# AntonXue/nn-sdp

Hardware: NVIDIA B200
Metric: queries/sec (clique LMI blocks assembled: value * cliques_per_query) (higher is better)
Workload: dtype f64

## Files before the change

### nn-sdp_b200/csrc/api.cu

```cuda
#include <math.h>
#include <stdarg.h>
#include <stdio.h>
#include <stdlib.h>
#include <string.h>

#include <algorithm>
#include <cmath>
#include <condition_variable>
#include <deque>
#include <functional>
#include <memory>
#include <mutex>
#include <thread>
#include <unordered_map>

#include <cuda.h>

#include "internal.h"

namespace nnsdp {

static thread_local std::string g_err;

void set_error(const char* fmt, ...) {
// ... 22 lines not shown
namespace {

struct DevBuf {
  void* p = nullptr;
  size_t cap = 0;
  int32_t ensure(size_t bytes) {
    if (bytes <= cap && p) return NNSDP_OK;
    if (p) cudaFree(p);
    p = nullptr;
    cap = 0;
    if (bytes == 0) bytes = 8;
    NN_CUDA(cudaMalloc(&p, bytes));
    cap = bytes;
    return NNSDP_OK;
  }
  void release() {
    if (p) cudaFree(p);
    p = nullptr;
    cap = 0;
  }
  template <class T>
  T* as() const {
    return reinterpret_cast<T*>(p);
  }
};

struct NetPerDev {
  int dev = -1;
  std::vector<DevBuf> M, Wt;
  DevBuf n, off, xoff, blk_of, Mptr, Wtptr, ldT, bias;
  NetDev nd{};
  void release() {
    for (auto& x : M) x.release();
    for (auto& x : Wt) x.release();
    n.release(); off.release(); xoff.release(); blk_of.release();
    Mptr.release(); Wtptr.release(); ldT.release(); bias.release();
  }
};

int round_up(int64_t v, int64_t m) { return (int)(((v + m - 1) / m) * m); }

}

struct nnsdp_net {
  nnsdp_ctx* ctx = nullptr;
  Shape sh;
  std::vector<int> ldT;
  std::vector<NetPerDev> per;
  int64_t max_block = 0;
  struct Cached {
    int dev_index;
    int64_t beta, Qcap, ring;
    int dense;
    nnsdp_batch* b;
  };
  mutable std::mutex cache_mu;
  mutable std::vector<Cached> cache;
};

namespace {

enum Stage {
  ST_BOUNDS = 0, ST_PREP = 1, ST_GRAM = 2, ST_EMIT = 3, ST_D2H = 4,
  ST_EMIT_FILL = 5, ST_EMIT_WINDOW = 6, ST_EMIT_EDGE = 7,
  ST_COUNT = 8
};

struct StageSpan {
  int stage;
  cudaEvent_t e0, e1;
};

}

namespace {

class WorkerPool {
 public:
  explicit WorkerPool(int n) {
    for (int i = 0; i < n; ++i) th_.emplace_back([this] { loop(); });
  }
  ~WorkerPool() {
    {
      std::lock_guard<std::mutex> l(m_);
      stop_ = true;
    }
    cv_.notify_all();
    for (auto& t : th_) t.join();
  }
  void submit(int group, std::function<void()> fn) {
    {
      std::lock_guard<std::mutex> l(m_);
      if ((int)pending_.size() <= group) pending_.resize(group + 1, 0);
      ++pending_[group];
      q_.emplace_back(group, std::move(fn));
    }
    cv_.notify_one();
  }
  void wait_group(int group) {
    std::unique_lock<std::mutex> l(m_);
    done_cv_.wait(l, [&] { return (int)pending_.size() <= group || pending_[group] == 0; });
  }
  void wait_all() {
    std::unique_lock<std::mutex> l(m_);
    done_cv_.wait(l, [&] {
      for (int p : pending_)
        if (p) return false;
      return true;
    });
    pending_.clear();
  }
  int size() const { return (int)th_.size(); }

 private:
  void loop() {
    for (;;) {
      std::pair<int, std::function<void()>> job;
      {
        std::unique_lock<std::mutex> l(m_);
        cv_.wait(l, [&] { return stop_ || !q_.empty(); });
        if (stop_ && q_.empty()) return;
        job = std::move(q_.front());
        q_.pop_front();
      }
      job.second();
      {
        std::lock_guard<std::mutex> l(m_);
        --pending_[job.first];
      }
      done_cv_.notify_all();
    }
  }
  std::vector<std::thread> th_;
  std::deque<std::pair<int, std::function<void()>>> q_;
  std::vector<int> pending_;
  std::mutex m_;
  std::condition_variable cv_, done_cv_;
  bool stop_ = false;
};

constexpr int GATHER_STAGES = 4;

}

struct nnsdp_batch {
  GatherPlan gp;
  std::vector<CliqueRanges> mats_host;
  DevBuf d_thin_idx, d_packed;
  double* h_packed = nullptr;
  size_t h_packed_doubles = 0;
  cudaEvent_t ev_packed[GATHER_STAGES] = {nullptr, nullptr, nullptr, nullptr};
  std::unique_ptr<WorkerPool> pool;
  std::vector<int> h_cnt;
  std::vector<int> h_pairs;
  std::vector<int64_t> pair_begin;
  DevBuf d_pairs;
  int64_t gather_bytes_dma = 0, gather_bytes_zeroed = 0, gather_bytes_thin = 0;
  nnsdp_ctx* ctx = nullptr;
  int dev_index = 0, dev = 0;
  const nnsdp_net* net = nullptr;
  const NetPerDev* nd = nullptr;
  int64_t beta = 0, Qcap = 0, ring = 0, Q = 0;
  bool dense = false;
  bool packed = false;
  PackedLayout lay;
  DevBuf d_bands;
  DevBuf d_tmaps, d_tmap_ok;
  int nbands = 0, band_max_m = 0;
  int64_t emitted_bytes = 0, packed_present_cells = 0;
  int64_t ring_zeroed = 0;
  std::vector<uint8_t> slot_bulk;
  std::vector<int> bulk_begin;
  std::vector<int64_t> bulk_entries;
  int64_t pass_entries = 0;
  std::vector<BulkItem> sel;
  std::vector<CholFront> chol;
  DevBuf d_chol;
  DevBuf ze_netv, ze_g, ze_rows, ze_part, ze_io, ze_err;
  nnsdp_sizes sz{};
  PlanHost plan;
  DevBuf d_tiles, d_strips, d_bulk, d_mats, d_panel, d_goff, d_ldG;
  std::vector<long long> goff;
  std::vector<int> ldG;
  long long gram_per_query = 0;
  DevBuf x1min, x1max, ymin, ymax, smin, smax, gin, gbnd, gsec, outS, outvec, outinvP, gout;
  DevBuf xmin, xmax, acxmin, acxmax, smin_c, smax_c;
  DevBuf d11, Md, T0, Bt, u, aff, part, act, cnt, Z11, Z1K, U;
  DevBuf gram, ringbuf, flags;
  DevBuf cr_rowsA, cr_rowsB, cr_bias, cr_prel, cr_preu, cr_du, cr_bu, cr_dl;
  DevBuf cr_keep_l, cr_keep_u;
  bool keep_preact = false, preact_valid = false;
  BatchDev bd{};
  GramDev gd{};
  PlanDev pd{};
  bool have_inputs = false, bounds_supplied = false, bounds_done = false, prepared = false;
  bool shared_gram = false;
  int bounds_method = 0;
  cudaStream_t st = nullptr, st_copy = nullptr;
  cudaEvent_t ev_start = nullptr, ev_stop = nullptr;
  cudaEvent_t ev_done[2] = {nullptr, nullptr}, ev_free[2] = {nullptr, nullptr};
  std::vector<StageSpan> spans;
  std::vector<cudaEvent_t> ev_pool;
  float stage_ms[ST_COUNT] = {};
  int64_t stage_launches[ST_COUNT] = {};

  cudaEvent_t get_event() {
    if (!ev_pool.empty()) {
      cudaEvent_t e = ev_pool.back();
      ev_pool.pop_back();
      return e;
    }
    cudaEvent_t e = nullptr;
    cudaEventCreate(&e);
    return e;
  }
  bool span_open = false;
  void span_begin(int stage, cudaStream_t s) {
    span_open = spans.size() < 16384;
    if (!span_open) return;
    StageSpan sp{stage, get_event(), get_event()};
    cudaEventRecord(sp.e0, s);
    spans.push_back(sp);
  }
  void span_end(cudaStream_t s, int launches) {
    if (!span_open) return;
    span_open = false;
    cudaEventRecord(spans.back().e1, s);
    stage_launches[spans.back().stage] += launches;
  }
  void resolve_spans() {
    for (auto& sp : spans) {
      float ms = 0.f;
      if (cudaEventElapsedTime(&ms, sp.e0, sp.e1) == cudaSuccess) {
        stage_ms[sp.stage] += ms;
        if (sp.stage >= 5 && sp.stage <= 7) stage_ms[3] += ms;
      }
      ev_pool.push_back(sp.e0);
      ev_pool.push_back(sp.e1);
    }
    spans.clear();
  }
  std::vector<DevBuf*> all_bufs() {
    return {&d_bands, &d_tmaps, &d_tmap_ok, &d_tiles, &d_strips, &d_bulk, &d_mats, &d_panel, &d_goff, &d_ldG, &d_chol, &ze_netv, &ze_g, &ze_rows, &ze_part, &ze_io, &ze_err, &x1min, &x1max, &ymin, &ymax, &smin, &smax,
            &gin, &gbnd, &gsec, &outS, &outvec, &outinvP, &gout, &xmin, &xmax, &acxmin, &acxmax,
            &smin_c, &smax_c, &d11, &Md, &T0, &Bt, &u, &aff, &part, &act, &cnt, &Z11, &Z1K, &U,
            &gram, &ringbuf, &flags, &cr_rowsA, &cr_rowsB, &cr_bias, &cr_prel, &cr_preu, &cr_du, &cr_bu, &cr_dl,
            &cr_keep_l, &cr_keep_u};
  }
};

namespace {

int32_t require_device() {
  int n = 0;
  cudaError_t e = cudaGetDeviceCount(&n);
  if (e != cudaSuccess || n <= 0) {
    cudaGetLastError();
    set_error("no CUDA device available (%s); this library has no CPU fallback",
              e == cudaSuccess ? "device count is 0" : cudaGetErrorString(e));
    return NNSDP_ERR_CUDA;
  }
  return NNSDP_OK;
}

int32_t upload(DevBuf& buf, const void* src, size_t bytes, cudaStream_t st) {
  NN_TRY(buf.ensure(bytes));
  if (bytes) NN_CUDA(cudaMemcpyAsync(buf.p, src, bytes, cudaMemcpyHostToDevice, st));
  return NNSDP_OK;
}

int32_t upload_cols(DevBuf& buf, const double* src, int64_t stride, int64_t len, int64_t Q,
                    cudaStream_t st, long long* dstride, const char* name) {
  NN_CHECK(src != nullptr, NNSDP_ERR_ARG, "query input '%s' is NULL", name);
  NN_CHECK(stride == 0 || stride >= len, NNSDP_ERR_ARG,
           "query input '%s': stride %lld < length %lld", name, (long long)stride, (long long)len);
  if (stride == 0 || Q == 1) {
    NN_TRY(buf.ensure((size_t)len * 8));
    if (len) NN_CUDA(cudaMemcpyAsync(buf.p, src, (size_t)len * 8, cudaMemcpyHostToDevice, st));
    *dstride = (stride == 0) ? 0 : len;
    return NNSDP_OK;
  }
  NN_TRY(buf.ensure((size_t)len * Q * 8));
  if (len == 0) {
    *dstride = 0;
    return NNSDP_OK;
  }
  if (stride == len)
    NN_CUDA(cudaMemcpyAsync(buf.p, src, (size_t)len * Q * 8, cudaMemcpyHostToDevice, st));
  else
    NN_CUDA(cudaMemcpy2DAsync(buf.p, (size_t)len * 8, src, (size_t)stride * 8, (size_t)len * 8,
                              (size_t)Q, cudaMemcpyHostToDevice, st));
  *dstride = len;
  return NNSDP_OK;
}

int32_t check_flags(nnsdp_batch* b, const char* where) {
  int h[4] = {0, 0, 0, 0};
  NN_CUDA(cudaMemcpyAsync(h, b->flags.p, sizeof(h), cudaMemcpyDeviceToHost, b->st));
  NN_CUDA(cudaStreamSynchronize(b->st));
  if (h[0] | h[1]) {
    NN_CUDA(cudaMemsetAsync(b->flags.p, 0, sizeof(h), b->st));
    if (h[0] & 1)
      NN_CHECK(false, NNSDP_ERR_ASSERT, "%s: acymin <= acymax violated (src/Qc/activ_bounded.jl:8)",
               where);
    if (h[0] & 2)
      NN_CHECK(false, NNSDP_ERR_ASSERT,
               "%s: 0 <= smin <= smax <= 1 violated (src/Qc/activ_sector.jl:14-16)", where);
    NN_CHECK(false, NNSDP_ERR_ASSERT,
             "%s: ykmin <= ykmax violated (src/Intervals/intervals_auto_lirpa.jl:60)", where);
  }
  return NNSDP_OK;
}

}

extern "C" {

const char* nnsdp_last_error(void) { return g_err.c_str(); }
int32_t nnsdp_version(void) { return 104; }

int32_t nnsdp_device_count(int32_t* count) {
  NN_CHECK(count != nullptr, NNSDP_ERR_ARG, "count is NULL");
  int n = 0;
  cudaError_t e = cudaGetDeviceCount(&n);
  if (e != cudaSuccess) {
    cudaGetLastError();
    n = 0;
  }
  *count = n;
  return NNSDP_OK;
}

int32_t nnsdp_ctx_create(int32_t ndev, const int32_t* dev_ids, nnsdp_ctx** out) {
  NN_CHECK(out != nullptr, NNSDP_ERR_ARG, "ctx output pointer is NULL");
  *out = nullptr;
  NN_CHECK(ndev >= 1, NNSDP_ERR_ARG, "ndev must be >= 1");
  NN_TRY(require_device());
  int avail = 0;
  NN_CUDA(cudaGetDeviceCount(&avail));
  std::unique_ptr<nnsdp_ctx> ctx(new nnsdp_ctx());
  for (int i = 0; i < ndev; ++i) {
    const int d = dev_ids ? dev_ids[i] : i;
    NN_CHECK(d >= 0 && d < avail, NNSDP_ERR_ARG, "device ordinal %d out of range (have %d)", d, avail);
    ctx->devs.push_back(d);
  }
  for (int d : ctx->devs) {
    NN_CUDA(cudaSetDevice(d));
    cudaStream_t s = nullptr;
    NN_CUDA(cudaStreamCreateWithFlags(&s, cudaStreamNonBlocking));
    ctx->streams.push_back(s);
  }
  *out = ctx.release();
  return NNSDP_OK;
}

int32_t nnsdp_ctx_destroy(nnsdp_ctx* ctx) {
  if (!ctx) return NNSDP_OK;
  for (size_t i = 0; i < ctx->streams.size(); ++i) {
    cudaSetDevice(ctx->devs[i]);
    cudaStreamSynchronize(ctx->streams[i]);
    cudaStreamDestroy(ctx->streams[i]);
  }
  delete ctx;
  return NNSDP_OK;
}

int32_t nnsdp_ctx_num_devices(const nnsdp_ctx* ctx, int32_t* ndev) {
  NN_CHECK(ctx && ndev, NNSDP_ERR_ARG, "NULL argument");
  *ndev = (int32_t)ctx->devs.size();
  return NNSDP_OK;
}

int32_t nnsdp_host_alloc(uint64_t bytes, void** ptr) {
  NN_CHECK(ptr != nullptr, NNSDP_ERR_ARG, "ptr is NULL");
  *ptr = nullptr;
  NN_TRY(require_device());
  NN_CUDA(cudaHostAlloc(ptr, bytes ? bytes : 8, cudaHostAllocPortable));
  return NNSDP_OK;
}

int32_t nnsdp_host_free(void* ptr) {
  if (ptr) NN_CUDA(cudaFreeHost(ptr));
  return NNSDP_OK;
}

static int32_t shape_from_xdims(int64_t K, const int64_t* xdims, Shape* sh) {
  NN_CHECK(xdims != nullptr, NNSDP_ERR_ARG, "xdims is NULL");
  NN_CHECK(K >= 2, NNSDP_ERR_ASSERT, "FeedFwdNet needs length(xdims) >= 3 (K >= 2)");
  NN_CHECK(K < 32768, NNSDP_ERR_ARG, "K too large");
  sh->K = (int)K;
  sh->n.assign(xdims, xdims + K + 1);
  for (auto v : sh->n) NN_CHECK(v >= 1 && v < (1 << 24), NNSDP_ERR_ARG, "bad layer width %lld", (long long)v);
  sh->off.assign(K + 1, 0);
  for (int b = 1; b <= K; ++b) sh->off[b] = sh->off[b - 1] + sh->n[b - 1];
  sh->xoff.assign(K + 2, 0);
  for (int b = 1; b <= K + 1; ++b) sh->xoff[b] = sh->xoff[b - 1] + sh->n[b - 1];
// ... 127 lines not shown
    }
  }
  if (ck_off) ck_off[ci.ck.size()] = o;
  if (d_off) d_off[2 * ci.ck.size()] = od;
  return NNSDP_OK;
}

int32_t nnsdp_cliques(const nnsdp_net* net, int64_t beta, int64_t* ck_off, int64_t* ck_idx,
                      int64_t* ck1_len, int64_t* d_off, int64_t* d_idx) {
  NN_CHECK(net != nullptr, NNSDP_ERR_ARG, "net is NULL");
  return cliques_out(net->sh, beta, ck_off, ck_idx, ck1_len, d_off, d_idx);
}

int32_t nnsdp_cliques_from_xdims(int64_t K, const int64_t* xdims, int64_t beta, int64_t* ck_off,
                                 int64_t* ck_idx, int64_t* ck1_len, int64_t* d_off, int64_t* d_idx) {
  Shape sh;
  NN_TRY(shape_from_xdims(K, xdims, &sh));
  return cliques_out(sh, beta, ck_off, ck_idx, ck1_len, d_off, d_idx);
}

static int32_t format_mats(const Shape& sh, int64_t beta, int32_t format, std::vector<CliqueRanges>* mats) {
  NN_CHECK(format >= 0 && format <= 2, NNSDP_ERR_ARG, "format must be NNSDP_FORMAT_BLOCKS, _DENSE_Z or _PACKED");
  mats->clear();
  if (format != NNSDP_FORMAT_BLOCKS) {
    CliqueRanges c;
    c.nseg = 1;
    c.lo[0] = 0;
    c.hi[0] = sh.Zdim - 1;
    mats->push_back(c);
  } else {
    CliqueInfoHost ci;
    NN_TRY(make_cliques_host(sh, beta, &ci));
    *mats = ci.ck;
  }
  return NNSDP_OK;
}

int32_t nnsdp_plan_stats(int64_t K, const int64_t* xdims, int64_t beta, int32_t dense_Z,
                         int64_t* tiles_per_prog, int64_t* entries_per_prog, int64_t* tile_rows,
                         int64_t* tile_cols) {
  NN_CHECK(tiles_per_prog && entries_per_prog, NNSDP_ERR_ARG, "NULL argument");
  Shape sh;
  NN_TRY(shape_from_xdims(K, xdims, &sh));
  nnsdp_sizes sz;
  NN_TRY(fill_sizes(sh, beta, &sz));
  std::vector<CliqueRanges> mats;
  NN_TRY(format_mats(sh, beta, dense_Z, &mats));
  PlanHost plan;
  PackedLayout lay;
  NN_TRY(build_plan(sh, beta, mats, true, &plan, dense_Z == NNSDP_FORMAT_PACKED ? &lay : nullptr));
  for (int i = 0; i < 8; ++i) tiles_per_prog[i] = entries_per_prog[i] = 0;
  for (const TileDev& t : plan.tiles) {
    tiles_per_prog[t.prog] += 1;
    entries_per_prog[t.prog] += (int64_t)t.nrows * t.ncols;
  }
  if (tile_rows) *tile_rows = plan.tile_rows;
  if (tile_cols) *tile_cols = plan.tile_cols;
  return NNSDP_OK;
}

int32_t nnsdp_plan_tiles(int64_t K, const int64_t* xdims, int64_t beta, int32_t dense_Z,
                         int64_t max_tiles, int32_t* tiles_out, int64_t* ntiles) {
  NN_CHECK(ntiles != nullptr, NNSDP_ERR_ARG, "NULL argument");
  Shape sh;
  NN_TRY(shape_from_xdims(K, xdims, &sh));
  nnsdp_sizes sz;
  NN_TRY(fill_sizes(sh, beta, &sz));
  std::vector<CliqueRanges> mats;
  NN_TRY(format_mats(sh, beta, dense_Z, &mats));
  PlanHost plan;
  PackedLayout lay;
  NN_TRY(build_plan(sh, beta, mats, true, &plan, dense_Z == NNSDP_FORMAT_PACKED ? &lay : nullptr));
  *ntiles = (int64_t)plan.tiles.size();
  if (tiles_out) {
    NN_CHECK(max_tiles >= *ntiles, NNSDP_ERR_ARG, "tiles_out too small");
    static_assert(sizeof(TileDev) == 11 * sizeof(int32_t), "TileDev layout");
    memcpy(tiles_out, plan.tiles.data(), plan.tiles.size() * sizeof(TileDev));
  }
  return NNSDP_OK;
}

int32_t nnsdp_plan_panel(int64_t K, const int64_t* xdims, int64_t beta, int32_t dense_Z, int64_t max_items,
                         int64_t* items_out, int64_t* nitems) {
  NN_CHECK(nitems != nullptr, NNSDP_ERR_ARG, "NULL argument");
  Shape sh;
  NN_TRY(shape_from_xdims(K, xdims, &sh));
  nnsdp_sizes sz;
  NN_TRY(fill_sizes(sh, beta, &sz));
  std::vector<CliqueRanges> mats;
  NN_TRY(format_mats(sh, beta, dense_Z, &mats));
  PlanHost plan;
  PackedLayout lay;
  NN_TRY(build_plan(sh, beta, mats, true, &plan, dense_Z == NNSDP_FORMAT_PACKED ? &lay : nullptr));
  *nitems = (int64_t)plan.panel.size();
  if (items_out) {
    NN_CHECK(max_items >= *nitems, NNSDP_ERR_ARG, "items_out too small");
    for (size_t i = 0; i < plan.panel.size(); ++i) {
      const StripDev& d = plan.panel[i];
      int64_t* o = items_out + 10 * i;
      o[0] = d.out_off; o[1] = d.ld; o[2] = d.row0; o[3] = d.nrows; o[4] = d.col0; o[5] = d.ncols;
      o[6] = d.grow0; o[7] = d.gcol0; o[8] = d.prog; o[9] = d.rblk;
    }
  }
  return NNSDP_OK;
}

int32_t nnsdp_gather_plan(int64_t K, const int64_t* xdims, int64_t beta, int32_t dense_Z, int64_t max_cells,
                          int32_t* cells_out, int64_t* ncells, int64_t max_thin, int64_t* thin_out,
                          int64_t* nthin, int32_t* usable) {
  NN_CHECK(ncells && nthin, NNSDP_ERR_ARG, "NULL argument");
  Shape sh;
  NN_TRY(shape_from_xdims(K, xdims, &sh));
  nnsdp_sizes sz;
  NN_TRY(fill_sizes(sh, beta, &sz));
  std::vector<CliqueRanges> mats;
  NN_CHECK(dense_Z == 0 || dense_Z == 1, NNSDP_ERR_ARG, "the host-gather plan exists for the dense formats only");
  NN_TRY(format_mats(sh, beta, dense_Z, &mats));
  PlanHost plan;
  NN_TRY(build_plan(sh, beta, mats, true, &plan));
  GatherPlan gp;
  NN_TRY(build_gather_plan(sh, beta, mats, plan, &gp));
  int64_t nc = 0;
  for (const GatherColSeg& cs : gp.colsegs) nc += (int64_t)cs.cells.size();
  *ncells = nc;
  *nthin = (int64_t)gp.thin_idx.size();
  if (usable) *usable = gp.usable ? 1 : 0;
  if (cells_out) {
    NN_CHECK(max_cells >= nc, NNSDP_ERR_ARG, "cells_out too small");
    int64_t i = 0;
    for (const GatherColSeg& cs : gp.colsegs)
      for (const GatherCell& c : cs.cells) {
        int32_t* o = cells_out + 8 * i++;
        o[0] = cs.mat; o[1] = c.row0; o[2] = c.nrows; o[3] = cs.col0; o[4] = cs.ncols;
        o[5] = c.kind; o[6] = c.blk; o[7] = c.pure_zero;
      }
  }
  if (thin_out) {
    NN_CHECK(max_thin >= *nthin, NNSDP_ERR_ARG, "thin_out too small");
    memcpy(thin_out, gp.thin_idx.data(), gp.thin_idx.size() * 8);
  }
  return NNSDP_OK;
}

int32_t nnsdp_batch_destroy(nnsdp_batch* b) {
  if (!b) return NNSDP_OK;
  cudaSetDevice(b->dev);
  if (b->st) cudaStreamSynchronize(b->st);
  if (b->st_copy) cudaStreamSynchronize(b->st_copy);
  b->resolve_spans();
  b->pool.reset();
  for (DevBuf* x : b->all_bufs()) x->release();
  b->d_thin_idx.release();
  b->d_packed.release();
  b->d_pairs.release();
  if (b->h_packed) cudaFreeHost(b->h_packed);
  for (cudaEvent_t e : b->ev_packed)
    if (e) cudaEventDestroy(e);
  for (cudaEvent_t e : b->ev_pool) cudaEventDestroy(e);
  for (cudaEvent_t e : {b->ev_start, b->ev_stop, b->ev_done[0], b->ev_done[1], b->ev_free[0], b->ev_free[1]})
    if (e) cudaEventDestroy(e);
  if (b->st) cudaStreamDestroy(b->st);
  if (b->st_copy) cudaStreamDestroy(b->st_copy);
  delete b;
  return NNSDP_OK;
}

int32_t nnsdp_batch_create(nnsdp_ctx* ctx, int32_t dev_index, const nnsdp_net* net, int64_t beta,
                           int64_t Qcap, int64_t ring_queries, int32_t dense_Z, nnsdp_batch** out) {
  NN_CHECK(out != nullptr, NNSDP_ERR_ARG, "batch output pointer is NULL");
  *out = nullptr;
  NN_CHECK(ctx && net, NNSDP_ERR_ARG, "NULL argument");
  NN_CHECK(net->ctx == ctx, NNSDP_ERR_ARG, "net was uploaded through a different ctx");
  NN_CHECK(dev_index >= 0 && dev_index < (int)ctx->devs.size(), NNSDP_ERR_ARG, "bad dev_index");
  NN_CHECK(Qcap >= 1 && Qcap < (1 << 30), NNSDP_ERR_ARG, "bad Qcap");
  NN_CHECK(ring_queries >= 0 && ring_queries <= 65535, NNSDP_ERR_ARG, "ring_queries must be in [0, 65535]");
  const Shape& sh = net->sh;
  nnsdp_batch* b = new nnsdp_batch();
  struct Guard {
    nnsdp_batch* b;
    ~Guard() { if (b) nnsdp_batch_destroy(b); }
  } guard{b};
  b->ctx = ctx;
  b->dev_index = dev_index;
  b->dev = ctx->devs[dev_index];
  b->net = net;
  b->nd = &net->per[dev_index];
  b->beta = beta;
  b->Qcap = Qcap;
  b->ring = std::min<int64_t>(ring_queries, Qcap);
  NN_CHECK(dense_Z >= 0 && dense_Z <= 2, NNSDP_ERR_ARG, "format must be NNSDP_FORMAT_BLOCKS, _DENSE_Z or _PACKED");
  b->dense = dense_Z == NNSDP_FORMAT_DENSE_Z;
  b->packed = dense_Z == NNSDP_FORMAT_PACKED;
  NN_TRY(fill_sizes(sh, beta, &b->sz));
  NN_CHECK(ring_queries == 0 || b->sz.sdim * b->sz.sdim * 8 + b->sz.n_out * 8 <= 200 * 1024, NNSDP_ERR_ARG,
           "n_in + n_out + 1 = %lld too large for the output-QC kernel (limit 160); bounds-only batches "
           "(ring_queries = 0) have no such limit", (long long)b->sz.sdim);
  NN_CUDA(cudaSetDevice(b->dev));
  NN_CUDA(cudaStreamCreateWithFlags(&b->st, cudaStreamNonBlocking));
  NN_CUDA(cudaStreamCreateWithFlags(&b->st_copy, cudaStreamNonBlocking));
  NN_CUDA(cudaEventCreate(&b->ev_start));
  NN_CUDA(cudaEventCreate(&b->ev_stop));
  for (int i = 0; i < 2; ++i) {
    NN_CUDA(cudaEventCreateWithFlags(&b->ev_done[i], cudaEventDisableTiming));
    NN_CUDA(cudaEventCreateWithFlags(&b->ev_free[i], cudaEventDisableTiming));
  }
  NN_TRY(b->flags.ensure(16));
  NN_CUDA(cudaMemsetAsync(b->flags.p, 0, 16, b->st));

  const int64_t Q = Qcap, ac = sh.acdim;
  NN_TRY(b->xmin.ensure((size_t)sh.xtot * Q * 8));
  NN_TRY(b->xmax.ensure((size_t)sh.xtot * Q * 8));
  NN_TRY(b->acxmin.ensure((size_t)ac * Q * 8));
  NN_TRY(b->acxmax.ensure((size_t)ac * Q * 8));
  NN_TRY(b->smin_c.ensure((size_t)ac * Q * 8));
  NN_TRY(b->smax_c.ensure((size_t)ac * Q * 8));
  if (b->ring > 0) {
    const int npart = (int)((ac + PREP_THREADS - 1) / PREP_THREADS);
    NN_TRY(b->d11.ensure((size_t)ac * Q * 8));
    NN_TRY(b->Md.ensure((size_t)ac * Q * 8));
    NN_TRY(b->T0.ensure((size_t)ac * Q * 8));
    NN_TRY(b->Bt.ensure((size_t)ac * Q * 8 * std::max<int64_t>(beta, 1)));
    NN_TRY(b->u.ensure((size_t)ac * Q * 8));
    NN_TRY(b->aff.ensure((size_t)sh.Zdim * Q * 8));
    NN_TRY(b->part.ensure((size_t)npart * Q * 8));
    NN_TRY(b->act.ensure((size_t)ac * Q * 4));
    NN_TRY(b->cnt.ensure((size_t)sh.K * Q * 4));
    NN_TRY(b->Z11.ensure((size_t)sh.n_in() * sh.n_in() * Q * 8));
    NN_TRY(b->Z1K.ensure((size_t)sh.n_in() * sh.n[sh.K - 1] * Q * 8));
    NN_TRY(b->U.ensure((size_t)sh.n_out() * sh.n[sh.K - 1] * Q * 8));
    b->bd.npart = npart;
    const long long go = gram_layout(sh, &b->goff, &b->ldG);
    b->gram_per_query = go;
    NN_TRY(upload(b->d_goff, b->goff.data(), b->goff.size() * 8, b->st));
    NN_TRY(upload(b->d_ldG, b->ldG.data(), b->ldG.size() * 4, b->st));
    NN_TRY(b->gram.ensure((size_t)go * b->ring * 8));
    std::vector<CliqueRanges> mats;
    NN_TRY(format_mats(sh, beta, dense_Z, &mats));
    const char* noclass = getenv("NNSDP_NO_TILE_CLASSES");
    NN_TRY(build_plan(sh, beta, mats, b->packed || !(noclass && noclass[0] == '1'), &b->plan,
                      b->packed ? &b->lay : nullptr));
    b->mats_host = mats;
    for (const BandDev& j : b->plan.bands) b->band_max_m = std::max(b->band_max_m, j.m);
    b->nbands = (int)b->plan.bands.size();
    NN_TRY(upload(b->d_bands, b->plan.bands.data(), b->plan.bands.size() * sizeof(BandDev), b->st));
    if (!b->packed) NN_TRY(build_gather_plan(sh, beta, mats, b->plan, &b->gp));
    if (const char* e = getenv("NNSDP_DENSE_GATHER"))
      if (e[0] == '1') b->gp.usable = false;
    if (b->gp.usable) {
      NN_TRY(upload(b->d_thin_idx, b->gp.thin_idx.data(), b->gp.thin_idx.size() * 8, b->st));
      for (int i = 0; i < GATHER_STAGES; ++i)
        NN_CUDA(cudaEventCreateWithFlags(&b->ev_packed[i], cudaEventDisableTiming));
    }
    NN_TRY(upload(b->d_tiles, b->plan.tiles.data(), b->plan.tiles.size() * sizeof(TileDev), b->st));
    NN_TRY(upload(b->d_mats, b->plan.mats.data(), b->plan.mats.size() * sizeof(MatDev), b->st));
    NN_TRY(b->ringbuf.ensure((size_t)b->plan.per_query_doubles * b->ring * 8));
    b->slot_bulk.assign((size_t)b->ring * sh.K, 0);
    auto is_bulk = [&](const StripDev& d) {
      return !b->packed && d.rblk >= 1 && d.rblk <= sh.K - 1 &&
             (d.prog == PROG_SAME || (d.prog == PROG_DIAG && !b->plan.band_inline));
    };
    std::vector<StripDev> strips, bulk;
    std::vector<std::vector<StripDev>> per_blk(sh.K);
    b->pass_entries = 0;
    b->bulk_entries.assign(sh.K, 0);
    for (const StripDev& d : b->plan.strips) {
      if (d.prog == PROG_ZERO) continue;
      if (is_bulk(d)) {
        per_blk[d.rblk].push_back(d);
        b->bulk_entries[d.rblk] += (int64_t)d.nrows * d.ncols;
      } else {
        strips.push_back(d);
        b->pass_entries += (int64_t)d.nrows * d.ncols;
      }
    }
    b->bulk_begin.assign(sh.K + 1, 0);
    for (int blk = 0; blk < sh.K; ++blk) {
      b->bulk_begin[blk] = (int)bulk.size();
      bulk.insert(bulk.end(), per_blk[blk].begin(), per_blk[blk].end());
    }
    b->bulk_begin[sh.K] = (int)bulk.size();
    for (int i = b->plan.n_fill; i < (int)b->plan.tiles.size(); ++i)
      b->pass_entries += (int64_t)b->plan.tiles[i].nrows * b->plan.tiles[i].ncols;
    for (const BandDev& j : b->plan.bands)
      if (j.ld > 0) b->pass_entries += (int64_t)j.m * (2 * beta + 1) - beta * (beta + 1);
    NN_TRY(upload(b->d_strips, strips.data(), strips.size() * sizeof(StripDev), b->st));
    NN_TRY(upload(b->d_bulk, bulk.data(), bulk.size() * sizeof(StripDev), b->st));
    b->pd.strips = b->d_strips.as<StripDev>();
    b->pd.bulk = b->d_bulk.as<StripDev>();
    b->pd.n_strips = (int)strips.size();
    b->pd.tiles = b->d_tiles.as<TileDev>();
    b->pd.mats = b->d_mats.as<MatDev>();
    b->pd.panel_desc = nullptr;
    b->pd.n_panel = 0;
    b->pd.fold = 0;
    {
      static const int panel_env = [] { const char* e = getenv("NNSDP_PANEL"); return e ? atoi(e) : 1; }();
      if (panel_env && !b->packed && !b->plan.panel.empty()) {
        const char* fold_env = getenv("NNSDP_PANEL_FOLD");
        const bool fold = !(fold_env && atoi(fold_env) == 0);
        std::vector<StripDev> panel;
        for (const StripDev& d : fold ? b->plan.panel_fold : b->plan.panel)
          if (d.prog != PROG_ZERO && (d.prog == PROG_RC || d.prog == PROG_CR || !is_bulk(d))) panel.push_back(d);
        NN_TRY(upload(b->d_panel, panel.data(), panel.size() * sizeof(StripDev), b->st));
        b->pd.panel_desc = b->d_panel.as<StripDev>();
        b->pd.n_panel = (int)panel.size();
        b->pd.fold = fold ? 1 : 0;
      }
    }
    b->pd.ntiles = (int)b->plan.tiles.size();
    b->pd.n_fill = b->plan.n_fill;
    b->pd.n_window = b->plan.n_window;
    b->pd.n_edge = b->plan.n_edge;
    b->pd.tile_rows = b->plan.tile_rows;
    b->pd.per_query = b->plan.per_query_doubles;
    b->pd.tmaps = nullptr;
    b->pd.tmap_ok = nullptr;
    if (b->plan.n_window > 0 && beta <= MAX_WINDOW_BETA) {
      typedef CUresult (*EncodeFn)(CUtensorMap*, CUtensorMapDataType, cuuint32_t, void*, const cuuint64_t*, const cuuint64_t*,
                                   const cuuint32_t*, const cuuint32_t*, CUtensorMapInterleave, CUtensorMapSwizzle,
                                   CUtensorMapL2promotion, CUtensorMapFloatOOBfill);
      void* fn = nullptr;
      cudaDriverEntryPointQueryResult qres;
      static const bool no_tma = [] { const char* e = getenv("NNSDP_NO_TMA"); return e && e[0] == '1'; }();
      if (!no_tma && cudaGetDriverEntryPoint("cuTensorMapEncodeTiled", &fn, cudaEnableDefault, &qres) == cudaSuccess && fn &&
          qres == cudaDriverEntryPointSuccess) {
        std::vector<CUtensorMap> maps(sh.K);
        std::vector<int> ok(sh.K, 0);
        bool any = false;
        for (int k = 0; k < sh.K; ++k) {
          if (sh.n[k + 1] % 2 != 0) continue;
          const cuuint64_t dims[2] = {(cuuint64_t)sh.n[k + 1], (cuuint64_t)sh.n[k]};
          const cuuint64_t strides[1] = {(cuuint64_t)sh.n[k + 1] * 8};
          const cuuint32_t box[2] = {(cuuint32_t)(128 + 2 * beta + 2), 32};
          const cuuint32_t estr[2] = {1, 1};
          const CUresult r = ((EncodeFn)fn)(&maps[k], CU_TENSOR_MAP_DATA_TYPE_FLOAT64, 2, b->nd->M[k].p, dims, strides, box, estr,
                                            CU_TENSOR_MAP_INTERLEAVE_NONE, CU_TENSOR_MAP_SWIZZLE_NONE,
                                            CU_TENSOR_MAP_L2_PROMOTION_L2_128B, CU_TENSOR_MAP_FLOAT_OOB_FILL_NONE);
          ok[k] = (r == CUDA_SUCCESS);
          any |= ok[k] != 0;
        }
        if (any) {
          static_assert(sizeof(CUtensorMap) == 128, "CUtensorMap is 128 bytes");
          NN_TRY(upload(b->d_tmaps, maps.data(), maps.size() * sizeof(CUtensorMap), b->st));
          NN_TRY(upload(b->d_tmap_ok, ok.data(), ok.size() * 4, b->st));
          NN_CUDA(cudaStreamSynchronize(b->st));
          b->pd.tmaps = b->d_tmaps.p;
          b->pd.tmap_ok = b->d_tmap_ok.as<int>();
        }
      } else {
        cudaGetLastError();
      }
    }
    b->pd.packed = b->plan.skip_absent ? 1 : 0;
    b->pd.band_inline = b->plan.band_inline ? 1 : 0;
    b->gd.scratch = b->gram.as<double>();
    b->gd.per_query = go;
    b->gd.goff = b->d_goff.as<long long>();
    b->gd.ldG = b->d_ldG.as<int>();
    b->gd.mirror = b->packed && b->plan.skip_absent ? 0 : 1;
  }
  NN_CUDA(cudaStreamSynchronize(b->st));
  guard.b = nullptr;
  *out = b;
  return NNSDP_OK;
}

int32_t nnsdp_batch_set_inputs(nnsdp_batch* b, int64_t Q, const nnsdp_query_inputs* in) {
  NN_CHECK(b && in, NNSDP_ERR_ARG, "NULL argument");
  NN_CHECK(Q >= 1 && Q <= b->Qcap, NNSDP_ERR_ARG, "Q = %lld outside [1, Qcap = %lld]", (long long)Q,
           (long long)b->Qcap);
  NN_CUDA(cudaSetDevice(b->dev));
  const Shape& sh = b->net->sh;
  const nnsdp_sizes& sz = b->sz;
  BatchDev& bd = b->bd;
  cudaStream_t st = b->st;
  b->have_inputs = false;
  b->bounds_done = b->prepared = false;
  b->preact_valid = false;
  b->Q = Q;
  bd.Q = (int)Q;
  bd.beta = (int)b->beta;
  bd.lamdim = sz.lamdim;
  bd.sdim = (int)sz.sdim;
  NN_TRY(upload_cols(b->x1min, in->x1min, in->x1min_stride, sz.n_in, Q, st, &bd.s_x1min, "x1min"));
  NN_TRY(upload_cols(b->x1max, in->x1max, in->x1max_stride, sz.n_in, Q, st, &bd.s_x1max, "x1max"));
  bd.x1min = b->x1min.as<double>();
  bd.x1max = b->x1max.as<double>();
  b->bounds_supplied = (in->ymin != nullptr);
  if (b->bounds_supplied) {
    NN_TRY(upload_cols(b->ymin, in->ymin, in->ymin_stride, sz.acdim, Q, st, &bd.s_ymin, "ymin"));
    NN_TRY(upload_cols(b->ymax, in->ymax, in->ymax_stride, sz.acdim, Q, st, &bd.s_ymax, "ymax"));
    NN_TRY(upload_cols(b->smin, in->smin, in->smin_stride, sz.acdim, Q, st, &bd.s_smin, "smin"));
    NN_TRY(upload_cols(b->smax, in->smax, in->smax_stride, sz.acdim, Q, st, &bd.s_smax, "smax"));
    bd.ymin = b->ymin.as<double>();
    bd.ymax = b->ymax.as<double>();
    bd.smin = b->smin.as<double>();
    bd.smax = b->smax.as<double>();
  } else {
    bd.ymin = b->xmin.as<double>() + sh.n_in();
    bd.ymax = b->xmax.as<double>() + sh.n_in();
    bd.s_ymin = bd.s_ymax = sh.xtot;
    bd.smin = b->smin_c.as<double>();
    bd.smax = b->smax_c.as<double>();
    bd.s_smin = bd.s_smax = sh.acdim;
  }
  if (b->ring > 0) {
    NN_TRY(upload_cols(b->gin, in->gamma_in, in->gamma_in_stride, sz.n_in, Q, st, &bd.s_gin, "gamma_in"));
    NN_TRY(upload_cols(b->gbnd, in->gamma_bnd, in->gamma_bnd_stride, sz.acdim, Q, st, &bd.s_gbnd, "gamma_bnd"));
    NN_TRY(upload_cols(b->gsec, in->gamma_sec, in->gamma_sec_stride, sz.secdim, Q, st, &bd.s_gsec, "gamma_sec"));
    bd.gin = b->gin.as<double>();
    bd.gbnd = b->gbnd.as<double>();
    bd.gsec = b->gsec.as<double>();
    bd.out_kind = in->out_kind;
    bd.outS = bd.outvec = bd.outinvP = bd.gout = nullptr;
    bd.s_outS = bd.s_outvec = bd.s_outinvP = bd.s_gout = 0;
    bd.has_s12 = bd.has_s22 = 0;
    switch (in->out_kind) {
      case NNSDP_OUT_SAFETY: {
        NN_TRY(upload_cols(b->outS, in->out_S, in->out_S_stride, sz.sdim * sz.sdim, Q, st, &bd.s_outS, "out_S"));
        bd.outS = b->outS.as<double>();
        const int64_t nq = in->out_S_stride == 0 ? 1 : Q, sd = sz.sdim, ni = sz.n_in, no = sz.n_out;
        for (int64_t q = 0; q < nq && !(bd.has_s12 && bd.has_s22); ++q) {
          const double* S = in->out_S + q * in->out_S_stride;
          for (int64_t c = ni; c < ni + no; ++c) {
            for (int64_t r = 0; r < ni; ++r) bd.has_s12 |= (S[r + c * sd] != 0.0);
            for (int64_t r = ni; r <= c; ++r) bd.has_s22 |= (S[r + c * sd] != 0.0);
          }
        }
        break;
      }
      case NNSDP_OUT_ELLIPSOID:
        NN_TRY(upload_cols(b->outinvP, in->out_invP, in->out_invP_stride, sz.n_out * sz.n_out, Q, st, &bd.s_outinvP, "out_invP"));
        bd.outinvP = b->outinvP.as<double>();
      case NNSDP_OUT_CIRCLE:
        bd.has_s22 = 1;
      case NNSDP_OUT_HPLANE:
        NN_TRY(upload_cols(b->outvec, in->out_vec, in->out_vec_stride, sz.n_out, Q, st, &bd.s_outvec, "out_vec"));
        NN_TRY(upload_cols(b->gout, in->gamma_out, in->gamma_out_stride, 1, Q, st, &bd.s_gout, "gamma_out"));
        bd.outvec = b->outvec.as<double>();
        bd.gout = b->gout.as<double>();
        break;
      default:
        NN_CHECK(false, NNSDP_ERR_ARG, "unrecognized out_kind %d (src/Qc/output.jl:95)", in->out_kind);
    }
    bd.d11 = b->d11.as<double>();
    bd.Md = b->Md.as<double>();
    bd.T0 = b->T0.as<double>();
    bd.Bt = b->Bt.as<double>();
    bd.u = b->u.as<double>();
    bd.aff = b->aff.as<double>();
    bd.part = b->part.as<double>();
    bd.act = b->act.as<int>();
    bd.cnt = b->cnt.as<int>();
    bd.Z11 = b->Z11.as<double>();
    bd.Z1K = b->Z1K.as<double>();
    bd.U = b->U.as<double>();
  }
  NN_CUDA(cudaStreamSynchronize(st));
  b->have_inputs = true;
  return NNSDP_OK;
}

int32_t nnsdp_batch_bounds(nnsdp_batch* b) {
  NN_CHECK(b != nullptr, NNSDP_ERR_ARG, "batch is NULL");
  NN_CHECK(b->have_inputs, NNSDP_ERR_STATE, "nnsdp_batch_bounds before nnsdp_batch_set_inputs");
  NN_CUDA(cudaSetDevice(b->dev));
  const Shape& sh = b->net->sh;
  const NetPerDev& nd = *b->nd;
  const int Q = (int)b->Q;
  double* xmin = b->xmin.as<double>();
  double* xmax = b->xmax.as<double>();
  b->preact_valid = false;
  b->span_begin(ST_BOUNDS, b->st);
  int launches = 0;
  int max_out = 0;
  for (int k = 1; k <= sh.K; ++k) max_out = std::max(max_out, (int)sh.n[k]);
  const int max_w = std::max(max_out, (int)sh.n[0]);
  int whole = ibp_chain_launch(nd.nd, max_w, b->bd.x1min, b->bd.s_x1min, b->bd.x1max, b->bd.s_x1max, xmin, xmax, sh.xtot,
                               b->acxmin.as<double>(), b->acxmax.as<double>(), b->smin_c.as<double>(),
                               b->smax_c.as<double>(), sh.acdim, Q, nullptr, b->st);
  if (whole == 0)
    whole = ibp_all_launch(nd.nd, max_out, b->bd.x1min, b->bd.s_x1min, b->bd.x1max, b->bd.s_x1max, xmin, xmax,
                           sh.xtot, b->acxmin.as<double>(), b->acxmax.as<double>(), b->smin_c.as<double>(),
                           b->smax_c.as<double>(), sh.acdim, Q, nullptr, b->st);
  NN_CHECK(whole >= 0, NNSDP_ERR_CUDA, "cooperative launch of the interval propagation failed: %s",
           cudaGetErrorString(cudaGetLastError()));
  launches += whole;
  if (whole == 0) {
    launches += launch_place_x1(b->bd.x1min, b->bd.s_x1min, b->bd.x1max, b->bd.s_x1max, xmin, xmax,
                                sh.xtot, (int)sh.n_in(), Q, b->st);
    for (int k = 0; k < sh.K; ++k) {
      const bool last = (k == sh.K - 1);
      launches += ibp_layer_launch(
          nd.M[k].as<double>(), (int)sh.n[k + 1], (int)sh.n[k], xmin + sh.xoff[k], xmax + sh.xoff[k],
          sh.xtot, xmin + sh.xoff[k + 1], xmax + sh.xoff[k + 1],
          last ? nullptr : b->acxmin.as<double>() + sh.noff(k + 1),
          last ? nullptr : b->acxmax.as<double>() + sh.noff(k + 1), sh.acdim, Q, last ? 0 : 1, 1,
          nullptr, b->st);
    }
    launches += launch_sector_minmax(sh.acdim * (long long)Q, b->acxmin.as<double>(),
                                     b->acxmax.as<double>(), b->smin_c.as<double>(),
                                     b->smax_c.as<double>(), b->st);
  }
  b->span_end(b->st, launches);
  NN_CUDA(cudaGetLastError());
  b->bounds_done = true;
  return NNSDP_OK;
}

int32_t nnsdp_batch_prepare(nnsdp_batch* b) {
  NN_CHECK(b != nullptr, NNSDP_ERR_ARG, "batch is NULL");
  NN_CHECK(b->have_inputs, NNSDP_ERR_STATE, "nnsdp_batch_prepare before nnsdp_batch_set_inputs");
  NN_CHECK(b->ring > 0, NNSDP_ERR_STATE, "batch was created without an output ring");
  NN_CHECK(b->bounds_supplied || b->bounds_done, NNSDP_ERR_STATE,
           "nnsdp_batch_prepare needs bounds: supply ymin/ymax/smin/smax or call nnsdp_batch_bounds");
  NN_CUDA(cudaSetDevice(b->dev));
  const Shape& sh = b->net->sh;
  const NetPerDev& nd = *b->nd;
  b->span_begin(ST_PREP, b->st);
  int launches = launch_prep(nd.nd, b->bd, b->flags.as<int>(), b->st);
  int max_rows = 0;
  for (int blk = 0; blk <= sh.K - 2; ++blk) max_rows = std::max(max_rows, (int)sh.n[blk]);
  const int all = affine_all_launch(nd.nd, sh.K, max_rows, b->bd.u, sh.acdim, b->bd.aff, sh.Zdim, (int)b->Q, b->st);
  launches += all;
  int lb0 = 0, lb1 = 0;
  if (all == 0) {
    auto fits = [&](int blk) {
      return sh.n[blk] >= 192 && sh.n[blk + 1] >= 128 && (sh.noff(blk + 1) & 1) == 0 && (sh.acdim & 1) == 0 &&
             (((uintptr_t)b->bd.u) & 15) == 0;
    };
    int best0 = 0, best1 = 0;
    for (int s = 0; s <= sh.K - 2;) {
      if (!fits(s)) { ++s; continue; }
      int e = s;
      while (e <= sh.K - 2 && fits(e)) ++e;
      if (e - s > best1 - best0) best0 = s, best1 = e;
      s = e;
    }
    int rows = 0;
    for (int blk = best0; blk < best1; ++blk) rows = std::max(rows, (int)sh.n[blk]);
    if (best1 - best0 >= 2 && dgemm_dmma_affine_layers_launch(nd.nd, best0, best1 - best0, rows, b->bd.u, sh.acdim, b->bd.aff,
                                                              sh.Zdim, (int)b->Q, b->st)) {
      lb0 = best0, lb1 = best1;
      ++launches;
    }
  }
  if (all == 0)
    for (int blk = 0; blk <= sh.K - 2; ++blk)
      if (blk < lb0 || blk >= lb1)
        launches += affine_layer_launch(nd.Wt[blk].as<double>(), b->net->ldT[blk], (int)sh.n[blk],
                                      (int)sh.n[blk + 1], b->bd.u + sh.noff(blk + 1), sh.acdim,
                                      b->bd.aff + sh.off[blk], sh.Zdim, (int)b->Q, b->st);
  b->span_end(b->st, launches);
  NN_CUDA(cudaGetLastError());
  b->h_cnt.resize((size_t)sh.K * b->Q);
  NN_CUDA(cudaMemcpyAsync(b->h_cnt.data(), b->cnt.p, b->h_cnt.size() * 4, cudaMemcpyDeviceToHost, b->st));
  NN_TRY(check_flags(b, "nnsdp_batch_prepare"));
  b->h_pairs.clear();
  b->pair_begin.assign((size_t)b->Q + 1, 0);
  for (int64_t q = 0; q < b->Q; ++q) {
    for (int blk = 0; blk <= sh.K - 2; ++blk)
      if (b->h_cnt[(size_t)q * sh.K + blk] > 0) {
        b->h_pairs.push_back((int)q);
        b->h_pairs.push_back(blk);
      }
    b->pair_begin[q + 1] = (int64_t)b->h_pairs.size() / 2;
  }
  NN_TRY(upload(b->d_pairs, b->h_pairs.data(), b->h_pairs.size() * 4, b->st));
  const BatchDev& bd = b->bd;
  b->shared_gram = b->Q > 1 && bd.s_gsec == 0 &&
                   (b->bounds_supplied ? (bd.s_smin == 0 && bd.s_smax == 0) : (bd.s_x1min == 0 && bd.s_x1max == 0));
  b->prepared = true;
  return NNSDP_OK;
}

static int32_t prepare_slots(nnsdp_batch* b, int64_t q0, int64_t nq, int64_t p0) {
  const int64_t per = b->plan.per_query_doubles;
  const int K = b->net->sh.K;
  if (p0 + nq > b->ring_zeroed) {
    NN_CUDA(cudaMemsetAsync(b->ringbuf.as<double>() + b->ring_zeroed * per, 0, (size_t)(p0 + nq - b->ring_zeroed) * per * 8,
                            b->st));
    std::fill(b->slot_bulk.begin() + b->ring_zeroed * K, b->slot_bulk.begin() + (p0 + nq) * K, 0);
    b->ring_zeroed = p0 + nq;
  }
  b->sel.clear();
  int64_t entries = b->pass_entries * nq;
  for (int64_t i = 0; i < nq; ++i) {
    const int64_t q = q0 + i;
    uint8_t* held = &b->slot_bulk[(size_t)(p0 + i) * K];
    for (int blk = 1; blk < K; ++blk) {
      const int first = b->bulk_begin[blk], count = b->bulk_begin[blk + 1] - first;
      if (count == 0) continue;
      const bool now = blk <= K - 2 ? b->h_cnt[(size_t)q * K + blk] > 0 : b->bd.has_s22 != 0;
      if (now || held[blk]) {
        b->sel.push_back({(int32_t)i, first, count});
        entries += b->bulk_entries[blk];
      }
      held[blk] = now;
    }
  }
  if (!b->packed) b->emitted_bytes += entries * 8;
  return NNSDP_OK;
}

static int32_t emit_pass(nnsdp_batch* b, const GramDev& gd, int q0, int nq, double* dst) {
  const NetPerDev& nd = *b->nd;
  NN_TRY(prepare_slots(b, q0, nq, (dst - b->ringbuf.as<double>()) / b->plan.per_query_doubles));
  int total = 0;
  for (int which = 0; which < 3; ++which) {
    b->span_begin(ST_EMIT_FILL + which, b->st);
    const int l = launch_emit(nd.nd, b->bd, gd, b->pd, q0, nq, dst, b->st, which, b->sel.data(), (int)b->sel.size());
    b->span_end(b->st, l);
    total += l;
  }
  if (b->nbands > 0) {
    b->span_begin(ST_EMIT_EDGE, b->st);
    const int l = launch_emit_band(nd.nd, b->bd, gd, b->d_bands.as<BandDev>(), b->nbands, b->band_max_m, b->pd.per_query,
                                   q0, nq, dst, b->st);
    b->span_end(b->st, l);
    total += l;
  }
  b->stage_launches[ST_EMIT] += total;
  const cudaError_t e = cudaGetLastError();
  if (e != cudaSuccess) {
    b->ring_zeroed = 0;
    return cuda_fail(e, "emitter pass", __FILE__, __LINE__);
  }
  return NNSDP_OK;
}

int32_t nnsdp_batch_emit(nnsdp_batch* b, int64_t q0, int64_t nq) {
  NN_CHECK(b != nullptr, NNSDP_ERR_ARG, "batch is NULL");
  NN_CHECK(b->prepared, NNSDP_ERR_STATE, "nnsdp_batch_emit before nnsdp_batch_prepare");
  NN_CHECK(q0 >= 0 && nq >= 1 && q0 + nq <= b->Q && nq <= b->ring, NNSDP_ERR_ARG,
           "bad query range [%lld, %lld) for Q = %lld, ring = %lld", (long long)q0,
           (long long)(q0 + nq), (long long)b->Q, (long long)b->ring);
  NN_CUDA(cudaSetDevice(b->dev));
  const NetPerDev& nd = *b->nd;
  GramDev gd = b->gd;
  b->span_begin(ST_GRAM, b->st);
  int l;
  if (b->shared_gram) {
    l = launch_gram(nd.nd, b->bd, gd, (int)b->net->max_block, 0, b->d_pairs.as<int>(), (int)b->pair_begin[1], b->st);
    gd.per_query = 0;
  } else {
    l = launch_gram(nd.nd, b->bd, gd, (int)b->net->max_block, (int)q0, b->d_pairs.as<int>() + 2 * b->pair_begin[q0],
                    (int)(b->pair_begin[q0 + nq] - b->pair_begin[q0]), b->st);
  }
  b->span_end(b->st, l > 0 ? l : 0);
  NN_CHECK(l >= 0, NNSDP_ERR_ARG, "a hidden layer of %lld neurons is too wide for the Gram kernel's grid", (long long)b->net->max_block);
  NN_CUDA(cudaGetLastError());
  NN_TRY(emit_pass(b, gd, (int)q0, (int)nq, b->ringbuf.as<double>()));
  return NNSDP_OK;
}

int32_t nnsdp_batch_sync(nnsdp_batch* b) {
  NN_CHECK(b != nullptr, NNSDP_ERR_ARG, "batch is NULL");
  NN_CUDA(cudaSetDevice(b->dev));
  NN_CUDA(cudaStreamSynchronize(b->st));
  NN_CUDA(cudaStreamSynchronize(b->st_copy));
  b->resolve_spans();
  return NNSDP_OK;
}

static int32_t gather_chunk(nnsdp_batch* b, int ci, int64_t q0, int64_t nq, int h, const double* dst,
                            double* host_out, int32_t flags) {
  const GatherPlan& gp = b->gp;
  const int64_t per = b->plan.per_query_doubles;
  const int64_t nthin = (int64_t)gp.thin_idx.size();
  const int sb = ci % GATHER_STAGES;
  const int K = b->net->sh.K;
  const bool prezeroed = (flags & NNSDP_RUN_HOST_PREZEROED) != 0;
  const int64_t chunk_cap = std::max<int64_t>(1, b->ring / 2);
  double* d_pk = b->d_packed.as<double>() + (int64_t)sb * chunk_cap * nthin;
  double* h_pk = b->h_packed + (int64_t)sb * chunk_cap * nthin;
  launch_pack_thin(dst, per, b->d_thin_idx.as<long long>(), nthin, d_pk, (int)nq, b->st);
  NN_CUDA(cudaEventRecord(b->ev_done[h], b->st));
  NN_CUDA(cudaStreamWaitEvent(b->st_copy, b->ev_done[h], 0));
  b->span_begin(ST_D2H, b->st_copy);
  if (nthin) NN_CUDA(cudaMemcpyAsync(h_pk, d_pk, (size_t)nq * nthin * 8, cudaMemcpyDeviceToHost, b->st_copy));
  NN_CUDA(cudaEventRecord(b->ev_packed[sb], b->st_copy));
  static const int dma_zero_pct = [] {
    const char* e = getenv("NNSDP_GATHER_DMA_ZERO_PCT");
    const int v = e ? atoi(e) : 20;
    return v < 0 ? 0 : (v > 100 ? 100 : v);
  }();
  auto dense_now = [&](const GatherCell& c, int64_t q) {
    return c.kind == GK_ALWAYS || (c.kind == GK_GRAM && b->h_cnt[q * K + c.blk] > 0) ||
           (c.kind == GK_S22 && b->bd.has_s22);
  };
  auto active = [&](const GatherCell& c, int64_t q) {
    if (dense_now(c, q)) return true;
    if (std::min<int64_t>(c.nrows, c.ncols_hint) < GATHER_MIN_RECT) return false;
    if (prezeroed) return false;
    const uint64_t hsh = ((uint64_t)q * 1315423911u) ^ ((uint64_t)c.row0 * 2654435761u) ^ ((uint64_t)c.col0_hint * 97u);
    return (int)((hsh >> 7) % 100) < dma_zero_pct;
  };
  for (int64_t q = q0; q < q0 + nq; ++q) {
    const double* src = dst + (q - q0) * per;
    double* out = host_out + q * per;
    for (const GatherColSeg& cs : gp.colsegs) {
      const MatDev& md = b->plan.mats[cs.mat];
      for (const GatherCell& c : cs.cells) {
        if (!active(c, q)) continue;
        const int64_t off = md.out_off + c.row0 + (int64_t)cs.col0 * md.ld;
        NN_CUDA(cudaMemcpy2DAsync(out + off, (size_t)md.ld * 8, src + off, (size_t)md.ld * 8,
                                  (size_t)c.nrows * 8, (size_t)cs.ncols, cudaMemcpyDeviceToHost, b->st_copy));
        b->gather_bytes_dma += (int64_t)c.nrows * cs.ncols * 8;
      }
    }
  }
  b->span_end(b->st_copy, 0);
  NN_CUDA(cudaEventRecord(b->ev_free[h], b->st_copy));
  b->gather_bytes_thin += nq * nthin * 8;
  const int nm = (int)b->plan.mats.size();
  cudaEvent_t ev = b->ev_packed[sb];
  const int dev = b->dev;
  for (int64_t q = q0; q < q0 + nq; ++q) {
    for (int m = 0; m < nm; ++m) {
      double* out = host_out + q * per;
      const double* pk = h_pk + (q - q0) * nthin;
      struct Run { int64_t off; int32_t nrows, ncols, ld; };
      std::vector<Run> runs;
      const MatDev& md = b->plan.mats[m];
      for (int s = gp.colseg_begin[m]; s < gp.colseg_begin[m + 1]; ++s) {
        const GatherColSeg& cs = gp.colsegs[s];
        int32_t run0 = -1, runlen = 0;
        auto flush = [&] {
          if (runlen > 0) {
            runs.push_back({md.out_off + run0 + (int64_t)cs.col0 * md.ld, runlen, cs.ncols, md.ld});
            b->gather_bytes_zeroed += (int64_t)runlen * cs.ncols * 8;
          }
          run0 = -1;
          runlen = 0;
        };
        for (const GatherCell& c : cs.cells) {
          const bool skip = active(c, q) || (prezeroed && c.pure_zero);
          if (skip) {
            flush();
            continue;
          }
          if (runlen > 0 && run0 + runlen == c.row0) {
            runlen += c.nrows;
          } else {
            flush();
            run0 = c.row0;
            runlen = c.nrows;
          }
        }
        flush();
      }
      const int64_t t0 = gp.thin_begin[m], t1 = gp.thin_begin[m + 1];
      const int64_t* idx = gp.thin_idx.data();
      b->pool->submit(ci, [=, runs = std::move(runs)] {
        for (const Run& r : runs)
          for (int32_t c = 0; c < r.ncols; ++c) memset(out + r.off + (int64_t)c * r.ld, 0, (size_t)r.nrows * 8);
        if (t1 > t0) {
          cudaSetDevice(dev);
          cudaEventSynchronize(ev);
          for (int64_t i = t0; i < t1; ++i) out[idx[i]] = pk[i];
        }
      });
    }
  }
  return NNSDP_OK;
}

extern "C" int32_t nnsdp_batch_bounds_crown(nnsdp_batch* b);

static int32_t run_impl(nnsdp_batch* b, double* host_out, uint8_t* present, int32_t flags) {
  NN_CHECK(b != nullptr, NNSDP_ERR_ARG, "batch is NULL");
  NN_CHECK(b->have_inputs, NNSDP_ERR_STATE, "nnsdp_batch_run before nnsdp_batch_set_inputs");
  NN_CHECK(b->ring > 0, NNSDP_ERR_STATE, "batch was created without an output ring");
  NN_CUDA(cudaSetDevice(b->dev));
  if (!b->bounds_supplied) NN_TRY(b->bounds_method == 1 ? nnsdp_batch_bounds_crown(b) : nnsdp_batch_bounds(b));
  NN_TRY(nnsdp_batch_prepare(b));
  const NetPerDev& nd = *b->nd;
  const int64_t per = b->plan.per_query_doubles;
  const int nhalf = (host_out && b->ring >= 2) ? 2 : 1;
  const int64_t chunk = (nhalf == 2) ? b->ring / 2 : b->ring;
  const bool sparse = host_out && !b->packed && b->gp.usable && !(flags & NNSDP_RUN_DENSE_COPY);
  b->gather_bytes_dma = b->gather_bytes_zeroed = b->gather_bytes_thin = 0;
  b->emitted_bytes = b->packed_present_cells = 0;
  const int K = b->net->sh.K;
  const size_t ncells = b->lay.cells.size();
  auto cell_present = [&](int64_t q, const PackedCell& c) {
    if (c.always) return true;
    return c.blk <= K - 2 ? b->h_cnt[(size_t)q * K + c.blk] > 0 : b->bd.has_s22 != 0;
  };
  int64_t zero_entries = 0;
  if (b->packed)
    for (int i = 0; i < b->plan.n_fill; ++i)
      if (b->plan.tiles[i].prog == PROG_ZERO) zero_entries += (int64_t)b->plan.tiles[i].nrows * b->plan.tiles[i].ncols;
  if (b->packed)
    for (int64_t q = 0; q < b->Q; ++q) {
      int64_t ent = b->lay.always_entries - zero_entries;
      for (size_t i = 0; i < ncells; ++i) {
        const PackedCell& c = b->lay.cells[i];
        const bool p = cell_present(q, c);
        if (present) present[(size_t)q * ncells + i] = p ? 1 : 0;
        if (!c.always && p) ent += b->plan.skip_absent ? b->lay.diag_entries[c.blk] : 0, ++b->packed_present_cells;
      }
      b->emitted_bytes += ent * 8;
    }
  if (sparse) {
    const size_t need = (size_t)GATHER_STAGES * chunk * b->gp.thin_idx.size();
    if (need > b->h_packed_doubles) {
      if (b->h_packed) cudaFreeHost(b->h_packed);
      b->h_packed = nullptr;
      b->h_packed_doubles = 0;
      NN_CUDA(cudaHostAlloc((void**)&b->h_packed, std::max<size_t>(need, 1) * 8, cudaHostAllocPortable));
      b->h_packed_doubles = need;
      NN_TRY(b->d_packed.ensure(std::max<size_t>(need, 1) * 8));
    }
    if (!b->pool) {
      int nt = (int)std::min<unsigned>(16u, std::max(1u, std::thread::hardware_concurrency()));
      if (const char* e = getenv("NNSDP_HOST_THREADS")) nt = std::max(1, atoi(e));
      b->pool.reset(new WorkerPool(nt));
    }
  }
  bool used[2] = {false, false};
  int h = 0, ci = 0;
  int32_t status = NNSDP_OK;
  for (int64_t q0 = 0; q0 < b->Q && status == NNSDP_OK; q0 += chunk, h = (h + 1) % nhalf, ++ci) {
    const int64_t nq = std::min(chunk, b->Q - q0);
    double* dst = b->ringbuf.as<double>() + (int64_t)h * chunk * per;
    GramDev gd = b->gd;
    if (b->shared_gram) gd.per_query = 0;
    else gd.scratch += (int64_t)h * chunk * gd.per_query;
    if (sparse && ci >= GATHER_STAGES) b->pool->wait_group(ci - GATHER_STAGES);
    if (host_out && used[h]) NN_CUDA(cudaStreamWaitEvent(b->st, b->ev_free[h], 0));
    if (!b->shared_gram || ci == 0) {
      b->span_begin(ST_GRAM, b->st);
      int l = b->shared_gram
                  ? launch_gram(nd.nd, b->bd, b->gd, (int)b->net->max_block, 0, b->d_pairs.as<int>(), (int)b->pair_begin[1], b->st)
                  : launch_gram(nd.nd, b->bd, gd, (int)b->net->max_block, (int)q0, b->d_pairs.as<int>() + 2 * b->pair_begin[q0],
                                (int)(b->pair_begin[q0 + nq] - b->pair_begin[q0]), b->st);
      b->span_end(b->st, l > 0 ? l : 0);
      NN_CHECK(l >= 0, NNSDP_ERR_ARG, "a hidden layer of %lld neurons is too wide for the Gram kernel's grid",
               (long long)b->net->max_block);
      NN_CUDA(cudaGetLastError());
    }
    status = emit_pass(b, gd, (int)q0, (int)nq, dst);
    if (status != NNSDP_OK) break;
    if (sparse) {
      status = gather_chunk(b, ci, q0, nq, h, dst, host_out, flags);
      used[h] = true;
    } else if (host_out && b->packed && !(flags & NNSDP_RUN_DENSE_COPY)) {
      NN_CUDA(cudaEventRecord(b->ev_done[h], b->st));
      NN_CUDA(cudaStreamWaitEvent(b->st_copy, b->ev_done[h], 0));
      b->span_begin(ST_D2H, b->st_copy);
      const int64_t alw = b->lay.always_doubles;
      if (alw == per)
        NN_CUDA(cudaMemcpyAsync(host_out + q0 * per, dst, (size_t)nq * per * 8, cudaMemcpyDeviceToHost, b->st_copy));
      else
        NN_CUDA(cudaMemcpy2DAsync(host_out + q0 * per, (size_t)per * 8, dst, (size_t)per * 8, (size_t)alw * 8, (size_t)nq,
                                  cudaMemcpyDeviceToHost, b->st_copy));
      b->gather_bytes_dma += nq * alw * 8;
      for (int64_t q = q0; q < q0 + nq; ++q)
        for (size_t i = 0; i < ncells; ++i) {
          const PackedCell& c = b->lay.cells[i];
          if (c.always || !cell_present(q, c)) continue;
          const int64_t cells_doubles = c.nrows * c.ncols;
          NN_CUDA(cudaMemcpyAsync(host_out + q * per + c.offset, dst + (q - q0) * per + c.offset, (size_t)cells_doubles * 8,
                                  cudaMemcpyDeviceToHost, b->st_copy));
          b->gather_bytes_dma += cells_doubles * 8;
        }
      b->span_end(b->st_copy, 0);
      NN_CUDA(cudaEventRecord(b->ev_free[h], b->st_copy));
      used[h] = true;
    } else if (host_out) {
      NN_CUDA(cudaEventRecord(b->ev_done[h], b->st));
      NN_CUDA(cudaStreamWaitEvent(b->st_copy, b->ev_done[h], 0));
      b->span_begin(ST_D2H, b->st_copy);
      NN_CUDA(cudaMemcpyAsync(host_out + q0 * per, dst, (size_t)nq * per * 8, cudaMemcpyDeviceToHost,
                              b->st_copy));
      b->span_end(b->st_copy, 0);
      NN_CUDA(cudaEventRecord(b->ev_free[h], b->st_copy));
      used[h] = true;
      b->gather_bytes_dma += nq * per * 8;
    }
  }
  if (b->pool) b->pool->wait_all();
  if (status != NNSDP_OK) {
    cudaStreamSynchronize(b->st);
    cudaStreamSynchronize(b->st_copy);
    return status;
  }
  NN_CUDA(cudaGetLastError());
  NN_CUDA(cudaStreamSynchronize(b->st));
  NN_CUDA(cudaStreamSynchronize(b->st_copy));
  b->resolve_spans();
  return NNSDP_OK;
}

int32_t nnsdp_batch_run_ex(nnsdp_batch* b, double* host_out, int32_t flags) { return run_impl(b, host_out, nullptr, flags); }

int32_t nnsdp_batch_run(nnsdp_batch* b, double* host_out) { return run_impl(b, host_out, nullptr, 0); }

int32_t nnsdp_batch_run_packed(nnsdp_batch* b, double* host_records, uint8_t* present, int32_t flags) {
  NN_CHECK(b != nullptr, NNSDP_ERR_ARG, "batch is NULL");
  NN_CHECK(b->packed, NNSDP_ERR_STATE, "the batch was not created with NNSDP_FORMAT_PACKED");
  return run_impl(b, host_records, present, flags);
}

int32_t nnsdp_batch_packed_stats(nnsdp_batch* b, int64_t* record_doubles, int64_t* ncells, int64_t* emitted_bytes,
                                 int64_t* d2h_bytes, int64_t* present_optional_cells) {
  NN_CHECK(b != nullptr, NNSDP_ERR_ARG, "batch is NULL");
  NN_CHECK(b->packed, NNSDP_ERR_STATE, "the batch was not created with NNSDP_FORMAT_PACKED");
  if (record_doubles) *record_doubles = b->lay.record_doubles;
  if (ncells) *ncells = (int64_t)b->lay.cells.size();
  if (emitted_bytes) *emitted_bytes = b->emitted_bytes;
  if (d2h_bytes) *d2h_bytes = b->gather_bytes_dma;
  if (present_optional_cells) *present_optional_cells = b->packed_present_cells;
  return NNSDP_OK;
}

int32_t nnsdp_batch_emit_stats(nnsdp_batch* b, int64_t* emitted_bytes) {
  NN_CHECK(b && emitted_bytes, NNSDP_ERR_ARG, "NULL argument");
  *emitted_bytes = b->emitted_bytes;
  return NNSDP_OK;
}

int32_t nnsdp_batch_gather_stats(nnsdp_batch* b, int64_t* dma_bytes, int64_t* thin_bytes,
                                 int64_t* zeroed_bytes, int32_t* sparse_usable) {
  NN_CHECK(b != nullptr, NNSDP_ERR_ARG, "batch is NULL");
  if (dma_bytes) *dma_bytes = b->gather_bytes_dma;
  if (thin_bytes) *thin_bytes = b->gather_bytes_thin;
  if (zeroed_bytes) *zeroed_bytes = b->gather_bytes_zeroed;
  if (sparse_usable) *sparse_usable = b->gp.usable ? 1 : 0;
  return NNSDP_OK;
}

int32_t nnsdp_batch_get_bounds(nnsdp_batch* b, double* xmin, double* xmax, double* acxmin,
                               double* acxmax, double* smin, double* smax) {
  NN_CHECK(b != nullptr, NNSDP_ERR_ARG, "batch is NULL");
  NN_CHECK(b->bounds_done, NNSDP_ERR_STATE, "bounds have not been computed on the device");
  NN_CUDA(cudaSetDevice(b->dev));
  const Shape& sh = b->net->sh;
  const size_t Q = (size_t)b->Q;
  auto get = [&](double* dst, const DevBuf& src, size_t len) -> int32_t {
    if (dst) NN_CUDA(cudaMemcpyAsync(dst, src.p, len * Q * 8, cudaMemcpyDeviceToHost, b->st));
    return NNSDP_OK;
  };
  NN_TRY(get(xmin, b->xmin, sh.xtot));
  NN_TRY(get(xmax, b->xmax, sh.xtot));
  NN_TRY(get(acxmin, b->acxmin, sh.acdim));
  NN_TRY(get(acxmax, b->acxmax, sh.acdim));
  NN_TRY(get(smin, b->smin_c, sh.acdim));
  NN_TRY(get(smax, b->smax_c, sh.acdim));
  NN_CUDA(cudaStreamSynchronize(b->st));
  return NNSDP_OK;
}

int32_t nnsdp_batch_get_slot(nnsdp_batch* b, int64_t slot, double* host_out) {
  NN_CHECK(b && host_out, NNSDP_ERR_ARG, "NULL argument");
  NN_CHECK(slot >= 0 && slot < b->ring, NNSDP_ERR_ARG, "slot out of range");
  NN_CUDA(cudaSetDevice(b->dev));
  const int64_t per = b->plan.per_query_doubles;
  NN_CUDA(cudaMemcpyAsync(host_out, b->ringbuf.as<double>() + slot * per, (size_t)per * 8,
                          cudaMemcpyDeviceToHost, b->st));
  NN_CUDA(cudaStreamSynchronize(b->st));
  return NNSDP_OK;
}

int32_t nnsdp_batch_get_affine(nnsdp_batch* b, double* aff_out) {
  NN_CHECK(b && aff_out, NNSDP_ERR_ARG, "NULL argument");
  NN_CHECK(b->prepared, NNSDP_ERR_STATE, "batch is not prepared");
  NN_CUDA(cudaSetDevice(b->dev));
  NN_CUDA(cudaMemcpyAsync(aff_out, b->aff.p, (size_t)b->net->sh.Zdim * b->Q * 8,
                          cudaMemcpyDeviceToHost, b->st));
  NN_CUDA(cudaStreamSynchronize(b->st));
  return NNSDP_OK;
}

int32_t nnsdp_batch_ring_ptr(nnsdp_batch* b, uint64_t* dev_ptr, int64_t* slot_doubles) {
  NN_CHECK(b != nullptr, NNSDP_ERR_ARG, "batch is NULL");
  if (dev_ptr) *dev_ptr = (uint64_t)(uintptr_t)b->ringbuf.p;
  if (slot_doubles) *slot_doubles = b->plan.per_query_doubles;
  return NNSDP_OK;
}

int32_t nnsdp_batch_ring_reset(nnsdp_batch* b) {
  NN_CHECK(b != nullptr, NNSDP_ERR_ARG, "batch is NULL");
  b->ring_zeroed = 0;
  return NNSDP_OK;
}

int32_t nnsdp_batch_event_record(nnsdp_batch* b, int32_t which) {
  NN_CHECK(b != nullptr, NNSDP_ERR_ARG, "batch is NULL");
  NN_CUDA(cudaSetDevice(b->dev));
  NN_CUDA(cudaEventRecord(which == 0 ? b->ev_start : b->ev_stop, b->st));
  return NNSDP_OK;
}

// ... 1430 lines not shown
```

### nn-sdp_b200/csrc/internal.h

```cpp
#pragma once

#include <cuda_runtime.h>
#include <stdint.h>

#include <string>
#include <vector>

#include "../../include/nnsdp_b200.h"

namespace nnsdp {

void set_error(const char* fmt, ...);
int32_t cuda_fail(cudaError_t e, const char* what, const char* file, int line);

#define NN_CUDA(call)                                                                \
  do {                                                                               \
    cudaError_t _e = (call);                                                         \
    if (_e != cudaSuccess) return ::nnsdp::cuda_fail(_e, #call, __FILE__, __LINE__); \
  } while (0)

#define NN_CHECK(cond, code, ...)      \
  do {                                 \
    if (!(cond)) {                     \
      ::nnsdp::set_error(__VA_ARGS__); \
      return (code);                   \
    }                                  \
  } while (0)

#define NN_TRY(expr)               \
  do {                             \
    int32_t _s = (expr);           \
    if (_s != NNSDP_OK) return _s; \
  } while (0)

struct Shape {
  int K = 0;
  std::vector<int64_t> n;
  std::vector<int64_t> off;
  std::vector<int64_t> xoff;
  int64_t Zdim = 0, acdim = 0, xtot = 0;
  int64_t n_in() const { return n[0]; }
  int64_t n_out() const { return n[K]; }
  int64_t noff(int b) const { return off[b] - n[0]; }
  int block_of(int64_t z) const {
    int b = 0;
    while (b < K && z >= off[b + 1]) ++b;
    return b;
  }
};

struct CliqueRanges {
  int nseg = 0;
  int64_t lo[2] = {0, 0}, hi[2] = {0, 0};
  int64_t size() const {
    int64_t s = 0;
    for (int i = 0; i < nseg; ++i) s += hi[i] - lo[i] + 1;
    return s;
  }
};

struct CliqueInfoHost {
  std::vector<CliqueRanges> ck;
  std::vector<std::vector<int64_t>> d1, d2;
};

int32_t make_cliques_host(const Shape& sh, int64_t beta, CliqueInfoHost* out);
int64_t lambda_dim(int64_t acdim, int64_t beta);
long long gram_layout(const Shape& sh, std::vector<long long>* goff, std::vector<int>* ldG);
int32_t fill_sizes(const Shape& sh, int64_t beta, nnsdp_sizes* out);

enum TileFlags : uint32_t {
  TF_AFF = 1u << 0,
  TF_SAME = 1u << 1,
  TF_1K = 1u << 2,
  TF_RC = 1u << 3,
  TF_CR = 1u << 4,
  TF_BAND = 1u << 5,
  TF_ALL = 0x3Fu,
  TF_UNIFORM = 1u << 8,
};

enum TileProg : int32_t {
  PROG_ZERO = 0, PROG_SAME = 1, PROG_RC = 2, PROG_CR = 3, PROG_MIXED = 4, PROG_GENERAL = 5,
  PROG_DIAG = 6, PROG_AFF = 7,
};

struct TileDev {
  int32_t mat;
  int32_t row0, nrows;
  int32_t col0, ncols;
  int32_t grow0;
  int32_t gcol0;
  uint32_t flags;
  int32_t rblk, cblk;
  int32_t prog;
};

struct alignas(16) StripDev {
  long long out_off;
  long long goff;
  int32_t ld, row0, nrows, col0;
  int32_t ncols, grow0, gcol0, prog;
  int32_t rblk, rl0, cl0, ldG;
};
static_assert(sizeof(StripDev) == 64, "StripDev must be 64 bytes");

struct MatDev {
  int64_t out_off;
  int32_t n;
  int32_t ld;
};

enum PackedKind : int32_t { PK_WINDOW = 1, PK_DIAG = 2, PK_BAND = 3, PK_RECT = 4 };
struct PackedCell {
  int32_t kind, blk;
  int64_t grow0, gcol0;
  int64_t nrows, ncols;
  int64_t offset;
  int32_t always;
};
struct PackedLayout {
  std::vector<PackedCell> cells;
  int64_t record_doubles = 0;
  int64_t always_doubles = 0;
  int64_t always_entries = 0;
  std::vector<int32_t> diag_cell;
  std::vector<int64_t> diag_entries;
};
struct BandDev {
  long long out_off;
  long long band_off;
  int ld, row0, col0;
  int g0, m, blk;
  int optional;
  int upper_only;
};

struct PlanHost {
  std::vector<StripDev> strips;
  std::vector<TileDev> tiles;
  std::vector<MatDev> mats;
  int64_t per_query_doubles = 0;
  int tile_rows = 0, tile_cols = 0;
  std::vector<BandDev> bands;
  bool band_inline = true;
  int n_fill = 0, n_window = 0, n_edge = 0;
  bool skip_absent = false;
  std::vector<StripDev> panel;
  std::vector<StripDev> panel_fold;
};

enum GatherKind : int32_t { GK_NONE = 0, GK_ALWAYS = 1, GK_GRAM = 2, GK_S22 = 3 };
constexpr int GATHER_MIN_RECT = 256;

struct GatherCell {
  int32_t row0, nrows;
  int32_t kind, blk;
  int32_t pure_zero;
  int32_t ncols_hint, col0_hint;
};
struct GatherColSeg {
  int32_t mat, col0, ncols;
  std::vector<GatherCell> cells;
};
struct GatherPlan {
  bool usable = false;
  std::vector<GatherColSeg> colsegs;
  std::vector<int32_t> colseg_begin;
  std::vector<int64_t> thin_idx;
  std::vector<int64_t> thin_begin;
  int64_t dense_always_doubles = 0;
};

int32_t build_plan(const Shape& sh, int64_t beta, const std::vector<CliqueRanges>& mats,
                   bool classify, PlanHost* plan, PackedLayout* packed = nullptr);
void unpack_record(const Shape& sh, int64_t beta, const PackedLayout& lay, const std::vector<CliqueRanges>& mats,
                   const double* record, const uint8_t* present, double* out);
int32_t build_gather_plan(const Shape& sh, int64_t beta, const std::vector<CliqueRanges>& mats,
                          const PlanHost& plan, GatherPlan* gp);

struct CholFront {
  long long out_off;
  long long g0;
  int n, npriv;
  int lead, tail;
};
int32_t build_chol_plan(const Shape& sh, const std::vector<CliqueRanges>& mats, std::vector<CholFront>* fronts);

struct NetDev {
  int K, n_in, n_out, Zdim, acdim, xtot;
  const int* n;
  const int* off;
  const int* xoff;
  const int* blk_of;
  const double* const* M;
  const double* const* Wt;
  const int* ldT;
  const double* bias_all;
};

struct BatchDev {
  int Q, beta;
  int out_kind, has_s22, has_s12;
  int sdim;
  long long lamdim;
  const double* x1min;   long long s_x1min;
  const double* x1max;   long long s_x1max;
  const double* ymin;    long long s_ymin;
  const double* ymax;    long long s_ymax;
  const double* smin;    long long s_smin;
  const double* smax;    long long s_smax;
  const double* gin;     long long s_gin;
  const double* gbnd;    long long s_gbnd;
  const double* gsec;    long long s_gsec;
  const double* outS;    long long s_outS;
  const double* outvec;  long long s_outvec;
  const double* outinvP; long long s_outinvP;
  const double* gout;    long long s_gout;
  double* d11;
  double* Md;
  double* T0;
  double* Bt;
  double* u;
  double* aff;
  double* part;
  int npart;
  int* act;
  int* cnt;
  double* Z11;
  double* Z1K;
  double* U;
};

struct GramDev {
  double* scratch;
  long long per_query;
  const long long* goff;
  const int* ldG;
  int mirror;
};

struct PlanDev {
  const StripDev* strips;
  const StripDev* bulk;
  int n_strips;
  const TileDev* tiles;
  const MatDev* mats;
  const StripDev* panel_desc;
  int n_panel;
  int fold;
  int ntiles;
  int n_fill, n_window, n_edge;
  int tile_rows;
  long long per_query;
  const void* tmaps;
  const int* tmap_ok;
  int packed;
  int band_inline;
};

int ibp_layer_launch(const double* Mk, int n_out_k, int n_in_k, const double* xin_min,
                     const double* xin_max, long long x_stride, double* xout_min, double* xout_max,
                     double* acx_min, double* acx_max, long long acx_stride, int Q, int relu,
                     int write_x, int* flag_bad, cudaStream_t st);
int affine_layer_launch(const double* Wt, int ldT, int n_rows, int n_neurons, const double* u,
                        long long u_stride, double* aff, long long aff_stride, int Q,
                        cudaStream_t st);
int affine_all_launch(const NetDev& nd, int K, int max_rows, const double* u, long long u_stride, double* aff,
                      long long aff_stride, int Q, cudaStream_t st);
int ibp_all_launch(const NetDev& nd, int max_out, const double* x1min, long long s_min, const double* x1max,
                   long long s_max, double* xmin, double* xmax, long long x_stride, double* acxmin, double* acxmax,
                   double* smin, double* smax, long long acx_stride, int Q, int* flag_bad, cudaStream_t st);
int dgemm_dmma_launch(const double* A, int lda, int M, int K, const double* B, long long ldb, double* C, long long ldc,
                      int N, int accumulate, cudaStream_t st);
int ibp_dmma_launch(const double* Mk, int n_out_k, int n_in_k, const double* xin_min, const double* xin_max,
                    long long x_stride, double* xout_min, double* xout_max, double* acx_min, double* acx_max,
                    long long acx_stride, int Q, int relu, int write_x, int* flag_bad, cudaStream_t st);
int dgemm_dmma_affine_layers_launch(const NetDev& nd, int b0, int nb, int max_rows, const double* u, long long u_stride,
                                    double* aff, long long aff_stride, int Q, cudaStream_t st);
int ibp_chain_launch(const NetDev& nd, int max_w, const double* x1min, long long s_min, const double* x1max,
                     long long s_max, double* xmin, double* xmax, long long x_stride, double* acxmin, double* acxmax,
                     double* smin, double* smax, long long acx_stride, int Q, int* flag_bad, cudaStream_t st);
int launch_sector_minmax(long long n, const double* acxmin, const double* acxmax, double* smin,
                         double* smax, cudaStream_t st);
int launch_place_x1(const double* x1min, long long s_min, const double* x1max, long long s_max,
                    double* xmin, double* xmax, long long xtot, int n_in, int Q, cudaStream_t st);
int launch_transpose_w(const double* Mk, int n_out_k, int n_in_k, double* Wt, int ldT,
                       cudaStream_t st);
int launch_prep(const NetDev& net, const BatchDev& b, int* err_flag, cudaStream_t st);
int launch_gram(const NetDev& net, const BatchDev& b, const GramDev& g, int max_n, int q0, const int* pairs,
                int npairs, cudaStream_t st);
struct BulkItem {
  int32_t slot, first, count;
};
constexpr int BULK_PER_LAUNCH = 512;
struct BulkSel {
  int32_t n;
  BulkItem item[BULK_PER_LAUNCH];
};
int launch_emit(const NetDev& net, const BatchDev& b, const GramDev& g, const PlanDev& plan,
                int q0, int nq, double* out, cudaStream_t st, int which, const BulkItem* sel, int nsel);

struct AffineDev {
  long long nvar, var_out, var_bnd, var_sec;
  long long acdim, lamdim, beta;
  int out_kind;
  const double *x1min, *x1max, *ymin, *ymax, *smin, *smax;
  long long s_x1min, s_x1max, s_ymin, s_ymax, s_smin, s_smax;
  const long long* col_ptr;
  const int* lo;
};
int launch_affine_count(const NetDev& net, const AffineDev& A, long long* counts, cudaStream_t st);
int launch_affine_fill(const NetDev& net, const AffineDev& A, const long long* offs, long long* ent,
                       long long* var, double* val, cudaStream_t st);
int launch_affine_z0(const NetDev& net, const BatchDev& b, const AffineDev& A, long long nent, int Q, double* z0,
                     cudaStream_t st);
int launch_affine_csc_count(const NetDev& net, const AffineDev& A, const long long* first, long long ngroups,
                            long long* counts, cudaStream_t st);
int launch_affine_csc_fill(const NetDev& net, const AffineDev& A, const long long* first, long long ngroups,
                           const long long* offs, long long* ent, double* val, cudaStream_t st);
long long scan_scratch_len(long long n);
int launch_scan_exclusive(long long* x, long long n, long long* sums, cudaStream_t st);
int launch_affine_group_starts(const long long* offs, long long nvar, long long ngroups, long long* starts,
                               cudaStream_t st);

int launch_eig_init(double* v, int Zdim, int Qc, int q_first, cudaStream_t st);
int launch_eig_mid(const NetDev& net, const BatchDev& b, int q_first, int Qc, const double* x,
                   const double* t, double* s1, double* y, cudaStream_t st);
int launch_eig_io(const NetDev& net, const BatchDev& b, int q_first, int Qc, const double* x, double* y,
                  cudaStream_t st);
int launch_eig_multidot(const double* V, const double* w, int n, int Qc, int nv, double* c, int c_ld,
                        cudaStream_t st);
int launch_eig_project(const double* V, double* w, int n, int Qc, int nv, const double* c, int c_ld,
                       cudaStream_t st);
int launch_eig_normalize(const double* w, double* dst, int n, int Qc, double* nrm, cudaStream_t st);
int gemm_acc_launch(const double* A, int lda, int M, int Kdim, const double* B, long long ldb,
                    double* C, long long ldc, int N, cudaStream_t st);
int gemm_set_launch(const double* A, int lda, int M, int Kdim, const double* B, long long ldb,
                    double* C, long long ldc, int N, cudaStream_t st);

int launch_crown_params(const double* l, const double* u, long long stride, int n, int Qc, double* d_u,
                        double* b_u, double* d_l, cudaStream_t st);
int launch_crown_post(const double* prel, const double* preu, const double* d_u, const double* b_u, const double* d_l,
                      long long par_stride, int n, int Qc, double* out_lo, double* out_hi, long long out_stride,
                      cudaStream_t st);
int launch_crown_row(const double* srcL, const double* srcU, long long src_row_stride, long long src_q_stride,
                     double* dst, long long dst_row_stride, int nrows, int Qc, int n, const double* d_u,
                     const double* b_u, const double* d_l, long long par_stride, const double* bias_k,
                     double* bias, cudaStream_t st);
int launch_crown_step(const double* Wt, int ldT, int M, int Kdim, const double* srcL, const double* srcU,
                      long long src_row_stride, long long src_q_stride, double* dst, long long ld, int nrows, int Rs,
                      int Qc, const double* d_u, const double* b_u, const double* d_l, long long par_stride,
                      const double* bias_k, double* bias, cudaStream_t st);
int launch_crown_init_bias(const double* bt, int nrows, int Qc, double* bias, cudaStream_t st);
int launch_crown_init_post(const double* Wt, int ldT, int n_in_k, const double* bias_k, const double* d_u,
                           const double* b_u, const double* d_l, long long par_stride, double* dst,
                           long long dst_row_stride, int nrows, int Rs, int row0, int Qc, double* bias,
                           cudaStream_t st);
int launch_crown_chain(const NetDev& net, int t, int post, int ntargets, int maxw, int Qc, const double* d_u,
                       const double* b_u, const double* d_l, long long par_stride, const double* x1min, long long s_min,
                       const double* x1max, long long s_max, int q_first, double* out_lo, double* out_hi,
                       long long out_stride, cudaStream_t st);
int launch_crown_concretize(const double* rowsL, const double* rowsU, long long row_stride, long long q_stride,
                            int nrows, int Rs, int row0, int Qc, int n0, const double* x1min, long long s_min,
                            const double* x1max, long long s_max, int q_first, const double* bias, double* out_lo,
                            double* out_hi, long long out_stride, int postprocess, cudaStream_t st);

constexpr int CHOL_NB = 32;
int launch_chol_trace(const double* ring, long long per, const CholFront* fronts, int nfronts, int nq, double* stats,
                      cudaStream_t st);
int launch_chol_front_init(double* ring, long long per, const CholFront& f, const CholFront* prev, int nq,
                           const double* taup, const int* failed, cudaStream_t st);
int launch_chol_panel(double* ring, long long per, const CholFront& f, int j0, int w, int nq, int* failed,
                      long long* fail_index, double* min_pivot, cudaStream_t st);

int launch_zerr_net(const NetDev& net, double* netv, cudaStream_t st);
int launch_zerr_query(const NetDev& net, const BatchDev& b, const Shape& sh, const double* const* Wt, const int* ldT,
                      const double* netv, double* g, double* rows, double* part, double* io, double gN, double uf,
                      double* err, cudaStream_t st);
constexpr int ZERR_THREADS = 256;

int launch_emit_band(const NetDev& net, const BatchDev& b, const GramDev& g, const BandDev* bands, int nbands,
                     int max_m, long long per_query, int q0, int nq, double* out, cudaStream_t st);
int launch_pack_thin(const double* ring, long long per_query, const long long* idx, long long nthin,
                     double* packed, int nq, cudaStream_t st);

constexpr int PREP_THREADS = 256;
constexpr int STRIP_ROWS = 512, STRIP_COLS = 8;
constexpr int AFFROW_COLS = 1024;
constexpr int MAX_WINDOW_BETA = 4;
constexpr int MAX_FAST_BETA = 8;

}
```

### nn-sdp_b200/csrc/kernels_emit.cu

```cuda
#include <stdlib.h>

#include <algorithm>

#include "internal.h"

namespace nnsdp {

namespace {

constexpr int ETHREADS = 256;
constexpr int SLOT_GROUP = 8;
constexpr int FAST_TR = 128, FAST_TC = 32, FAST_NCOL = 16;
constexpr int MAX_TAPS = 2 * MAX_FAST_BETA + 1;
constexpr int MAX_TC = 32;

struct QView {
  const double* Md;
  const double* T0;
  const double* Bt;
  const double* gbnd;
  const double* aff;
  const double* Z11;
  const double* Z1K;
  const double* U;
  const int* cnt;
  const double* G;
};

__device__ __forceinline__ QView make_view(const NetDev& net, const BatchDev& b, const GramDev& g,
                                           int q, int slot) {
  const long long acdim = net.acdim;
  const int K = net.K, n0 = net.n_in;
  QView v;
  v.Md = b.Md + (long long)q * acdim;
  v.T0 = b.T0 + (long long)q * acdim;
  v.Bt = b.Bt + (long long)q * b.beta * acdim;
  v.gbnd = b.gbnd + q * b.s_gbnd;
  v.aff = b.aff + (long long)q * net.Zdim;
  v.Z11 = b.Z11 + (long long)q * n0 * n0;
  v.Z1K = b.Z1K + (long long)q * n0 * net.n[K - 1];
  v.U = b.U + (long long)q * net.n_out * net.n[K - 1];
  v.cnt = b.cnt + (long long)q * K;
  v.G = g.scratch + (long long)slot * g.per_query;
  return v;
}

__device__ __forceinline__ double m_coef(const double* Md, const double* Bt, long long acdim, int j,
                                         int c) {
  if (j == c) return Md[j];
  const int t = j > c ? j - c : c - j;
  return Bt[(long long)(t - 1) * acdim + (j < c ? j : c)];
}

__device__ __forceinline__ double band_term(const double* T0, const double* gbnd, const double* Bt,
                                            long long acdim, int jr, int jc) {
  if (jr == jc) return __dadd_rn(__dmul_rn(-2.0, T0[jr]), __dmul_rn(-2.0, gbnd[jr]));
  const int d = jr > jc ? jr - jc : jc - jr;
  return __dmul_rn(-2.0, Bt[(long long)(d - 1) * acdim + (jr < jc ? jr : jc)]);
}

__device__ __forceinline__ void emit_mixed(const NetDev& net, const BatchDev& b, const GramDev& g,
                                           const TileDev& t, const MatDev& mat, const QView& v,
                                           double* __restrict__ o, int tr, int cg, int ncg,
                                           double* smem) {
  const int K = net.K, n0 = net.n_in, beta = b.beta, ntap = 2 * beta + 1;
  const long long acdim = net.acdim;
  const uint32_t flags = t.flags;
  const int Br = t.rblk, Bc = t.cblk;
  const int rl0 = t.grow0 - net.off[Br], cl0 = t.gcol0 - net.off[Bc];
  const int jr0 = t.grow0 - n0, jc0 = t.gcol0 - n0;
  const bool same = (Br == Bc) && (flags & TF_SAME);
  const bool gram = same && Br <= K - 2 && v.cnt[Br] > 0;
  const bool z11 = same && Br == 0;
  const bool s22 = same && Br == K - 1 && b.has_s22;
  const bool k1a = (flags & TF_1K) && b.has_s12 && Br == 0 && Bc == K - 1;
  const bool k1b = (flags & TF_1K) && b.has_s12 && Bc == 0 && Br == K - 1;
  const bool rc = (flags & TF_RC) && Br <= K - 2 && Bc >= 1;
  const bool cr = (flags & TF_CR) && Bc <= K - 2 && Br >= 1;
  const bool band = (flags & TF_BAND) && Br >= 1 && Bc >= 1;
  const int Lr0 = rc ? net.off[Br + 1] - n0 : 0, nLr = rc ? net.n[Br + 1] : 0;
  const int Lc0 = cr ? net.off[Bc + 1] - n0 : 0, nLc = cr ? net.n[Bc + 1] : 0;
  double* coefRC = smem;
  double* coefCR = smem + MAX_TC * MAX_TAPS;

  __syncthreads();
  if (rc)
    for (int i = threadIdx.x; i < t.ncols * ntap; i += ETHREADS) {
      const int c = i / ntap, jc = jc0 + c, j = jc - beta + i % ntap;
      coefRC[i] = (j >= Lr0 && j < Lr0 + nLr) ? m_coef(v.Md, v.Bt, acdim, j, jc) : 0.0;
    }
  if (cr)
    for (int i = threadIdx.x; i < t.nrows * ntap; i += ETHREADS) {
      const int r = i / ntap, jr = jr0 + r, j = jr - beta + i % ntap;
      coefCR[i] = (j >= Lc0 && j < Lc0 + nLc) ? m_coef(v.Md, v.Bt, acdim, j, jr) : 0.0;
    }
  __syncthreads();
  if (tr >= t.nrows) return;

  const int rl = rl0 + tr, jr = jr0 + tr;
  const double* Gp = gram ? v.G + g.goff[Br] + rl : nullptr;
  const int ldG = gram ? g.ldG[Br] : 0;
  const double* WtR = rc ? net.Wt[Br] + rl : nullptr;
  const int ldTR = rc ? net.ldT[Br] : 0;
  const double* Wc0 = cr ? net.M[Bc] : nullptr;
  const double* WK = net.M[K - 1];
  const int n_out = net.n_out;
  const int cr_lo = cr ? max(0, Lc0 - (jr - beta)) : 0;
  const int cr_hi = cr ? min(ntap - 1, Lc0 + nLc - 1 - (jr - beta)) : -1;
  const double* myCR = coefCR + tr * ntap;

  for (int c = cg; c < t.ncols; c += ncg) {
    const int cl = cl0 + c, jc = jc0 + c;
    double val = 0.0;
    if (gram) val += Gp[(long long)cl * ldG];
    if (z11) val += v.Z11[rl + cl * n0];
    if (s22) {
      const int lo = rl < cl ? rl : cl, hi = rl < cl ? cl : rl;
      double s = 0.0;
      for (int m = 0; m < n_out; ++m)
        s = fma(WK[m + (long long)lo * n_out], v.U[m + (long long)hi * n_out], s);
      val += s;
    }
    if (k1a) val += v.Z1K[rl + (long long)cl * n0];
    if (k1b) val += v.Z1K[cl + (long long)rl * n0];
    double f1 = 0.0, f2 = 0.0;
    if (rc) {
      const int jb = jc - beta;
      const int lo = max(0, Lr0 - jb), hi = min(ntap - 1, Lr0 + nLr - 1 - jb);
      const double* w = WtR + (long long)(jb - Lr0) * ldTR;
      const double* cf = coefRC + c * ntap;
      for (int tt = lo; tt <= hi; ++tt) f1 = fma(w[(long long)tt * ldTR], cf[tt], f1);
    }
    if (cr) {
      const double* w = Wc0 + (long long)cl * nLc + (jr - beta - Lc0);
      for (int tt = cr_lo; tt <= cr_hi; ++tt) f2 = fma(w[tt], myCR[tt], f2);
    }
    val += f1 + f2;
    if (band) {
      const int d = jr > jc ? jr - jc : jc - jr;
      if (d <= beta) val = __dadd_rn(val, band_term(v.T0, v.gbnd, v.Bt, acdim, jr, jc));
    }
    o[(long long)c * mat.ld] = val;
  }
}

__device__ __forceinline__ void emit_general(const NetDev& net, const BatchDev& b, const GramDev& g,
                                             const TileDev& t, const MatDev& mat, const QView& v,
                                             double* __restrict__ o, int tr, int cg, int ncg) {
  if (tr >= t.nrows) return;
  const int K = net.K, n0 = net.n_in, a = net.Zdim - 1, beta = b.beta;
  const long long acdim = net.acdim;
  const uint32_t flags = t.flags;
  const int gr = t.grow0 + tr;
  const int Br = net.blk_of[gr];
  const int rl = gr - (Br < K ? net.off[Br] : a);
  const int jr = (gr >= n0 && gr < a) ? gr - n0 : -1;
  const bool r_feeds = (Br <= K - 2);
  const int Lr0 = r_feeds ? net.off[Br + 1] - n0 : 0;
  const int nLr = r_feeds ? net.n[Br + 1] : 0;
  const double* WtR = r_feeds ? net.Wt[Br] + rl : nullptr;
  const int ldTR = r_feeds ? net.ldT[Br] : 0;
  const double* WK = net.M[K - 1];
  const int n_out = net.n_out;

  for (int c = cg; c < t.ncols; c += ncg) {
    const int gc = t.gcol0 + c;
    double val = 0.0;
    if (gr == a || gc == a) {
      val = v.aff[gr == a ? gc : gr];
    } else {
      const int Bc = net.blk_of[gc];
      const int cl = gc - net.off[Bc];
      const int jc = gc >= n0 ? gc - n0 : -1;
      if ((flags & TF_SAME) && Br == Bc) {
        if (Br <= K - 2 && v.cnt[Br] > 0) val += v.G[g.goff[Br] + rl + (long long)cl * g.ldG[Br]];
        if (Br == 0) val += v.Z11[rl + cl * n0];
        if (Br == K - 1 && b.has_s22) {
          const int lo = rl < cl ? rl : cl, hi = rl < cl ? cl : rl;
          double s = 0.0;
          for (int m = 0; m < n_out; ++m)
            s = fma(WK[m + (long long)lo * n_out], v.U[m + (long long)hi * n_out], s);
          val += s;
        }
      }
      if ((flags & TF_1K) && b.has_s12) {
        if (Br == 0 && Bc == K - 1) val += v.Z1K[rl + (long long)cl * n0];
        if (Bc == 0 && Br == K - 1) val += v.Z1K[cl + (long long)rl * n0];
      }
      double f1 = 0.0, f2 = 0.0;
      if ((flags & TF_RC) && r_feeds && jc >= 0) {
        const int jlo = max(Lr0, jc - beta), jhi = min(Lr0 + nLr - 1, jc + beta);
        for (int j = jlo; j <= jhi; ++j)
          f1 = fma(WtR[(long long)(j - Lr0) * ldTR], m_coef(v.Md, v.Bt, acdim, j, jc), f1);
      }
      if ((flags & TF_CR) && Bc <= K - 2 && jr >= 0) {
        const int Lc0 = net.off[Bc + 1] - n0, nLc = net.n[Bc + 1];
        const double* Wc = net.M[Bc] + (long long)cl * nLc;
        const int jlo = max(Lc0, jr - beta), jhi = min(Lc0 + nLc - 1, jr + beta);
        for (int j = jlo; j <= jhi; ++j)
          f2 = fma(Wc[j - Lc0], m_coef(v.Md, v.Bt, acdim, j, jr), f2);
      }
      val += f1 + f2;
      if ((flags & TF_BAND) && jr >= 0 && jc >= 0) {
        const int d = jr > jc ? jr - jc : jc - jr;
        if (d <= beta) val = __dadd_rn(val, band_term(v.T0, v.gbnd, v.Bt, acdim, jr, jc));
      }
    }
    o[(long long)c * mat.ld] = val;
  }
}

template <int BETA, bool FULL>
__device__ __forceinline__ void emit_rc(const NetDev& net, const BatchDev& b, const PlanDev& plan,
                                        const TileDev& t, const MatDev& mat, int q0, int slot0,
                                        int nslots, double* __restrict__ out, double* smem) {
  constexpr int NTAP = 2 * BETA + 1;
  constexpr int PB = BETA + (BETA & 1);
  constexpr int RS = FAST_TC + PB;
  constexpr int QS = (BETA + 1) * RS;
  const int n0 = net.n_in;
  const long long acdim = net.acdim;
  const int Br = t.rblk;
  const int tr = threadIdx.x & (FAST_TR - 1), cg = threadIdx.x / FAST_TR;
  const int rl = t.grow0 - net.off[Br] + tr;
  const int jc0 = t.gcol0 - n0;
  const int Lr0 = net.off[Br + 1] - n0, nLr = net.n[Br + 1];

  for (int i = threadIdx.x; i < nslots * QS; i += ETHREADS) {
    const int s = i / QS, rem = i - s * QS, d = rem / RS, e = rem - d * RS;
    const long long idx = (long long)jc0 - PB + e;
    double v = 0.0;
    if (idx >= 0 && idx < acdim) {
      const long long q = q0 + slot0 + s;
      v = d == 0 ? b.Md[q * acdim + idx] : b.Bt[q * BETA * acdim + (long long)(d - 1) * acdim + idx];
    }
    smem[i] = v;
  }
  __syncthreads();
  if (tr >= t.nrows) return;

  const int cbase = cg * FAST_NCOL;
  double w[FAST_NCOL + NTAP - 1];
  {
    const double* WtR = net.Wt[Br] + rl;
    const int ldTR = net.ldT[Br];
    const int jb = jc0 + cbase - BETA;
#pragma unroll
    for (int i = 0; i < FAST_NCOL + NTAP - 1; ++i) {
      const int j = jb + i;
      w[i] = (j >= Lr0 && j < Lr0 + nLr) ? WtR[(long long)(j - Lr0) * ldTR] : 0.0;
    }
  }
  const long long ld = mat.ld;
  double* o0 = out + (long long)slot0 * plan.per_query + mat.out_off + (t.row0 + tr) + (long long)(t.col0 + cbase) * ld;
  const int ncl = t.ncols - cbase;
  for (int s = 0; s < nslots; ++s, o0 += plan.per_query) {
    const double* cf = smem + s * QS + cbase;
    double h[BETA + 1][BETA > 0 ? BETA : 1];
#pragma unroll
    for (int d = 1; d <= BETA; ++d)
#pragma unroll
      for (int k = 0; k < d; ++k) h[d][k] = cf[d * RS + PB - d + k];
    double* o = o0;
#pragma unroll
    for (int c = 0; c < FAST_NCOL; c += 2) {
      double x[BETA + 1], y[BETA + 1];
#pragma unroll
      for (int d = 0; d <= BETA; ++d) {
        const double2 v = *reinterpret_cast<const double2*>(cf + d * RS + PB + c);
        x[d] = v.x;
        y[d] = v.y;
      }
      double f = 0.0, g = 0.0;
#pragma unroll
      for (int tt = 0; tt < BETA; ++tt) {
        f = fma(w[c + tt], h[BETA - tt][0], f);
        g = fma(w[c + 1 + tt], (BETA - tt >= 2) ? h[BETA - tt][1] : x[BETA - tt], g);
      }
      f = fma(w[c + BETA], x[0], f);
      g = fma(w[c + 1 + BETA], y[0], g);
#pragma unroll
      for (int d = 1; d <= BETA; ++d) {
        f = fma(w[c + BETA + d], x[d], f);
        g = fma(w[c + 1 + BETA + d], y[d], g);
      }
      if (FULL || c < ncl) o[0] = f;
      if (FULL || c + 1 < ncl) o[ld] = g;
      o += 2 * ld;
#pragma unroll
      for (int d = 1; d <= BETA; ++d)
#pragma unroll
        for (int k = 0; k < d; ++k) h[d][k] = (k + 2 < d) ? h[d][k + 2] : (k + 2 == d ? x[d] : y[d]);
    }
  }
}

__host__ __device__ constexpr int CR_LDW(int beta) { return FAST_TR + 2 * beta + 2; }

__device__ __forceinline__ void tma_load_tile_2d(double* smem_dst, unsigned long long* mbar, const void* tmap, int c0,
                                                 int c1, unsigned bytes) {
  const unsigned bar = (unsigned)__cvta_generic_to_shared(mbar);
  const unsigned dst = (unsigned)__cvta_generic_to_shared(smem_dst);
  if (threadIdx.x == 0) {
    asm volatile("mbarrier.init.shared::cta.b64 [%0], 1;\n" ::"r"(bar));
    asm volatile("fence.mbarrier_init.release.cluster;\n" ::: "memory");
    asm volatile("mbarrier.arrive.expect_tx.shared::cta.b64 _, [%0], %1;\n" ::"r"(bar), "r"(bytes) : "memory");
    asm volatile(
        "cp.async.bulk.tensor.2d.shared::cluster.global.mbarrier::complete_tx::bytes [%0], [%1, {%2, %3}], [%4];\n" ::"r"(dst),
        "l"(tmap), "r"(c0), "r"(c1), "r"(bar)
        : "memory");
  }
  __syncthreads();
  unsigned done = 0, spins = 0;
  while (!done) {
    asm volatile("{\n.reg .pred p;\nmbarrier.try_wait.parity.shared::cta.b64 p, [%1], 0;\nselp.u32 %0, 1, 0, p;\n}\n"
                 : "=r"(done)
                 : "r"(bar)
                 : "memory");
    if (!done && ++spins > (1u << 24)) __trap();
  }
}

template <int BETA>
__device__ __forceinline__ void emit_cr(const NetDev& net, const BatchDev& b, const PlanDev& plan,
                                        const TileDev& t, const MatDev& mat, int q0, int slot0,
                                        int nslots, double* __restrict__ out, double* smem, unsigned long long* mbar) {
  constexpr int NTAP = 2 * BETA + 1;
  constexpr int LDW = CR_LDW(BETA);
  const int n0 = net.n_in;
  const long long acdim = net.acdim;
  const int Bc = t.cblk;
  const int tr = threadIdx.x & (FAST_TR - 1), cg = threadIdx.x / FAST_TR;
  const int jr0 = t.grow0 - n0, jr = jr0 + tr;
  const int cl0 = t.gcol0 - net.off[Bc];
  const int Lc0 = net.off[Bc + 1] - n0, nLc = net.n[Bc + 1];
  int adj = 0;
  if (plan.tmaps && plan.tmap_ok[Bc]) {
    const int c0 = jr0 - BETA - Lc0;
    adj = c0 & 1;
    tma_load_tile_2d(smem, mbar, (const char*)plan.tmaps + 128 * Bc, c0 - adj, cl0, (unsigned)(FAST_TC * LDW * 8));
  } else {
    const double* Wc0 = net.M[Bc] + (long long)cl0 * nLc;
    for (int i = threadIdx.x; i < t.ncols * LDW; i += ETHREADS) {
      const int c = i / LDW, ii = i - c * LDW;
      const int j = jr0 - BETA + ii;
      smem[i] = (j >= Lc0 && j < Lc0 + nLc) ? Wc0[(long long)c * nLc + (j - Lc0)] : 0.0;
    }
    __syncthreads();
  }
  if (tr >= t.nrows) return;
  const int cbase = cg * FAST_NCOL;
  const long long ld = mat.ld;
  double* o0 = out + (long long)slot0 * plan.per_query + mat.out_off + (t.row0 + tr) + (long long)(t.col0 + cbase) * ld;
  const int ncl = min(FAST_NCOL, t.ncols - cbase);
  const double* ws0 = smem + cbase * LDW + tr + adj;
  const double* Md = b.Md + (long long)(q0 + slot0) * acdim;
  const double* Bt = b.Bt + (long long)(q0 + slot0) * BETA * acdim;
  const long long pq = plan.per_query;
  int s = 0;
  for (; s + 2 <= nslots; s += 2, o0 += 2 * pq, Md += 2 * acdim, Bt += 2 * BETA * acdim) {
    double cf0[NTAP], cf1[NTAP];
#pragma unroll
    for (int tt = 0; tt < NTAP; ++tt) {
      const int j = jr - BETA + tt;
      const bool in = j >= Lc0 && j < Lc0 + nLc;
      cf0[tt] = in ? m_coef(Md, Bt, acdim, j, jr) : 0.0;
      cf1[tt] = in ? m_coef(Md + acdim, Bt + BETA * acdim, acdim, j, jr) : 0.0;
    }
    double* o = o0;
    const double* ws = ws0;
#pragma unroll 4
    for (int c = 0; c < ncl; ++c, o += ld, ws += LDW) {
      double f0 = 0.0, f1 = 0.0;
#pragma unroll
      for (int tt = 0; tt < NTAP; ++tt) {
        const double w = ws[tt];
        f0 = fma(w, cf0[tt], f0);
        f1 = fma(w, cf1[tt], f1);
      }
      o[0] = f0;
      o[pq] = f1;
    }
  }
  if (s < nslots) {
    double cf[NTAP];
#pragma unroll
    for (int tt = 0; tt < NTAP; ++tt) {
      const int j = jr - BETA + tt;
      cf[tt] = (j >= Lc0 && j < Lc0 + nLc) ? m_coef(Md, Bt, acdim, j, jr) : 0.0;
    }
    double* o = o0;
    const double* ws = ws0;
#pragma unroll 4
    for (int c = 0; c < ncl; ++c, o += ld, ws += LDW) {
      double f = 0.0;
#pragma unroll
      for (int tt = 0; tt < NTAP; ++tt) f = fma(ws[tt], cf[tt], f);
      *o = f;
    }
  }
}

__device__ __forceinline__ double s22_entry(const double* WK, const double* U, int n_out, int rl, int cl) {
  const int lo = rl < cl ? rl : cl, hi = rl < cl ? cl : rl;
  double acc = 0.0;
  for (int m = 0; m < n_out; ++m)
    acc = fma(WK[m + (long long)lo * n_out], U[m + (long long)hi * n_out], acc);
  return acc;
}

#ifndef NNSDP_FILL_MINB
#define NNSDP_FILL_MINB 6
#endif
template <bool BAND_INLINE>
__device__ __forceinline__ void fill_strip(const NetDev& net, const BatchDev& b, const GramDev& g, const PlanDev& plan,
                                           const StripDev* desc, int slot, int q0, double* __restrict__ out) {
  const int4* dp = reinterpret_cast<const int4*>(desc);
  const int4 d0 = __ldg(dp), d1 = __ldg(dp + 1), d2 = __ldg(dp + 2);
  const int tid = threadIdx.x;
  const long long out_off = ((long long)(unsigned)d0.x) | ((long long)d0.y << 32);
  const long long ld = d1.x;
  const int row0 = d1.y, nrows = d1.z, col0 = d1.w, ncols = d2.x, prog = d2.w;
  const int row_end = row0 + nrows;
  double* o = out + (long long)slot * plan.per_query + out_off;
  int lg = 5;
  while ((1 << lg) < ETHREADS && (1 << lg) < nrows + 3) ++lg;
  const int TR = 1 << lg;
  const int tr = tid & (TR - 1), cg = tid >> lg, ncg = ETHREADS >> lg;
  double* col = o + (col0 + cg) * ld;
  const long long cstep = (long long)ncg * ld;
#define NNSDP_STRIP_LOOP(VALUE)                                                     \
  for (int c = cg; c < ncols; c += ncg, col += cstep) {                               \
    int r = row0 - (int)(((size_t)(col + row0) >> 3) & 3) + tr;                       \
    if (r >= row0 && r < row_end) col[r] = (VALUE);                                   \
    for (r += TR; r < row_end; r += TR) col[r] = (VALUE);                             \
  }
  const int q = q0 + slot, K = net.K;
  const int grow0 = d2.y, gcol0 = d2.z;
  if (prog == PROG_AFF) {
    const double* aff = b.aff + (long long)q * net.Zdim;
    if (nrows == 1 && grow0 == net.Zdim - 1) {
      for (int c = tid; c < ncols; c += ETHREADS) o[row0 + (col0 + c) * ld] = aff[gcol0 + c];
    } else {
      aff += grow0 - row0;
      NNSDP_STRIP_LOOP(aff[r])
    }
    return;
  }
  const int4 d3 = __ldg(dp + 3);
  const int Br = d3.x, rl0 = d3.y, cl0 = d3.z, ldG = d3.w;
  const long long goff = ((long long)(unsigned)d0.z) | ((long long)d0.w << 32);
  const bool copy = Br <= K - 2 && b.cnt[(long long)q * K + Br] > 0;
  const bool s22 = Br == K - 1 && b.has_s22;
  if (plan.packed && !copy && !s22) return;
  const double* WK = net.M[K - 1];
  const double* U = b.U + (long long)q * net.n_out * net.n[K - 1];
  const double* G = g.scratch + (long long)slot * g.per_query + goff + rl0;
  if (BAND_INLINE && prog == PROG_DIAG) {
    const int beta = b.beta;
    const long long acdim = net.acdim;
    const int jr_base = grow0 - net.n_in - row0, jc0 = gcol0 - net.n_in;
    const double* T0 = b.T0 + (long long)q * acdim;
    const double* Bt = b.Bt + (long long)q * beta * acdim;
    const double* gbnd = b.gbnd + q * b.s_gbnd;
    const double* Gc = G + (long long)(cl0 + cg) * ldG;
    const long long gstep = (long long)ncg * ldG;
    for (int c = cg; c < ncols; c += ncg, col += cstep, Gc += gstep) {
      const int jc = jc0 + c;
      int r = row0 - (int)(((size_t)(col + row0) >> 3) & 3) + tr;
      for (; r < row_end; r += TR) {
        if (r < row0) continue;
        double v = copy ? Gc[r] : (s22 ? s22_entry(WK, U, net.n_out, rl0 + r, cl0 + c) : 0.0);
        const int d = jr_base + r - jc;
        if (d >= -beta && d <= beta) {
          v = 0.0 + v;
          v += 0.0;
          v = __dadd_rn(v, band_term(T0, gbnd, Bt, acdim, jc + d, jc));
        }
        col[r] = v;
      }
    }
  } else if (copy) {
    const double* Gc = G + (long long)(cl0 + cg) * ldG;
    const long long gstep = (long long)ncg * ldG;
    for (int c = cg; c < ncols; c += ncg, col += cstep, Gc += gstep) {
      int r = row0 - (int)(((size_t)(col + row0) >> 3) & 3) + tr;
      if (r >= row0 && r < row_end) col[r] = Gc[r];
      for (r += TR; r < row_end; r += TR) col[r] = Gc[r];
    }
  } else if (s22) {
    NNSDP_STRIP_LOOP(s22_entry(WK, U, net.n_out, rl0 + r, cl0 + c))
  } else {
    NNSDP_STRIP_LOOP(0.0)
  }
#undef NNSDP_STRIP_LOOP
}

template <bool BAND_INLINE>
__global__ void __launch_bounds__(ETHREADS, NNSDP_FILL_MINB)
emit_fill_kernel(NetDev net, BatchDev b, GramDev g, PlanDev plan, int q0, int nq,
                 double* __restrict__ out) {
  fill_strip<BAND_INLINE>(net, b, g, plan, plan.strips + blockIdx.x, blockIdx.y, q0, out);
}

template <bool BAND_INLINE>
__global__ void __launch_bounds__(ETHREADS, NNSDP_FILL_MINB)
emit_fill_kernel(NetDev net, BatchDev b, GramDev g, PlanDev plan, int q0, BulkSel sel, double* __restrict__ out) {
  const BulkItem it = sel.item[blockIdx.y];
  if ((int)blockIdx.x >= it.count) return;
  fill_strip<BAND_INLINE>(net, b, g, plan, plan.bulk + it.first + blockIdx.x, it.slot, q0, out);
}

template <int BETA>
__global__ void __launch_bounds__(ETHREADS, 4)
emit_window_kernel(NetDev net, BatchDev b, PlanDev plan, int tile0, int q0, int nq, int group, int group_major,
                   double* __restrict__ out) {
  constexpr int RC_DOUBLES = SLOT_GROUP * (BETA + 1) * (FAST_TC + BETA + 1), CR_DOUBLES = FAST_TC * CR_LDW(BETA);
  __shared__ __align__(128) double smem[RC_DOUBLES > CR_DOUBLES ? RC_DOUBLES : CR_DOUBLES];
  __shared__ __align__(8) unsigned long long mbar;
  const int ngroups = (nq + group - 1) / group;
  const int ti = group_major ? blockIdx.x % plan.n_window : blockIdx.x / ngroups;
  const int gi = group_major ? blockIdx.x / plan.n_window : blockIdx.x % ngroups;
  const TileDev t = plan.tiles[tile0 + ti];
  const MatDev mat = plan.mats[t.mat];
  const int slot0 = gi * group;
  const int nslots = min(group, nq - slot0);
  if (t.prog == PROG_RC) {
    if (t.ncols == FAST_TC) emit_rc<BETA, true>(net, b, plan, t, mat, q0, slot0, nslots, out, smem);
    else emit_rc<BETA, false>(net, b, plan, t, mat, q0, slot0, nslots, out, smem);
  } else {
    emit_cr<BETA>(net, b, plan, t, mat, q0, slot0, nslots, out, smem, &mbar);
  }
}

constexpr int EDGE_DOUBLES = MAX_TC * MAX_TAPS + 128 * MAX_TAPS;

__device__ __forceinline__ void emit_edge_tile(const NetDev& net, const BatchDev& b, const GramDev& g,
                                               const PlanDev& plan, const TileDev& t, const MatDev& mat, int q0,
                                               int slot0, int nslots, double* __restrict__ out, double* smem) {
  int TR = 1;
  while (TR < t.nrows) TR <<= 1;
  if (TR > ETHREADS) TR = ETHREADS;
  const int tr = threadIdx.x % TR, cg = threadIdx.x / TR, ncg = ETHREADS / TR;
  const long long tile_off = mat.out_off + (t.row0 + tr) + (long long)t.col0 * mat.ld;
  const bool uniform = (t.flags & TF_UNIFORM) != 0 && t.nrows * t.ncols > 512;
  if (uniform) {
    for (int s = 0; s < nslots; ++s) {
      const QView v = make_view(net, b, g, q0 + slot0 + s, slot0 + s);
      double* o = out + (long long)(slot0 + s) * plan.per_query + tile_off;
      emit_mixed(net, b, g, t, mat, v, o, tr, cg, ncg, smem);
    }
    return;
  }
  int TC = 1;
  while (TC < t.ncols && TC < ncg) TC <<= 1;
  const int per = TR * TC;
  const int spar = ETHREADS / per;
  const int sub = threadIdx.x / per, cg2 = (threadIdx.x % per) / TR;
  for (int s = sub; s < nslots; s += spar) {
    const QView v = make_view(net, b, g, q0 + slot0 + s, slot0 + s);
    double* o = out + (long long)(slot0 + s) * plan.per_query + tile_off;
    emit_general(net, b, g, t, mat, v, o, tr, cg2, TC);
  }
}

__global__ void __launch_bounds__(ETHREADS, 4)
emit_edge_kernel(NetDev net, BatchDev b, GramDev g, PlanDev plan, int tile0, int q0, int nq,
                 int group, double* __restrict__ out) {
  __shared__ double smem[EDGE_DOUBLES];
  const TileDev t = plan.tiles[tile0 + blockIdx.x];
  const MatDev mat = plan.mats[t.mat];
  const int slot0 = blockIdx.y * group;
  emit_edge_tile(net, b, g, plan, t, mat, q0, slot0, min(group, nq - slot0), out, smem);
}

template <int BETA, bool FOLD>
__global__ void __launch_bounds__(ETHREADS, 4)
emit_panel_kernel(NetDev net, BatchDev b, GramDev g, PlanDev plan, int q0, int nq, int group, double* __restrict__ out) {
  constexpr int RC_DOUBLES = SLOT_GROUP * (BETA + 1) * (FAST_TC + BETA + 1), CR_DOUBLES = FAST_TC * CR_LDW(BETA);
  constexpr int WIN_DOUBLES = RC_DOUBLES > CR_DOUBLES ? RC_DOUBLES : CR_DOUBLES;
  static_assert(WIN_DOUBLES >= EDGE_DOUBLES, "the edge tiles stage their band coefficients in the same buffer");
  __shared__ __align__(128) double smem[WIN_DOUBLES];
  __shared__ __align__(8) unsigned long long mbar;
  const int batch = group >> 8;
  group &= 255;
  const int gb = batch / group;
  const int per_batch = plan.n_panel * gb;
  const int sb = blockIdx.x / per_batch, rem = blockIdx.x - sb * per_batch;
  const int slot_lo = sb * batch, slot_hi = min(nq, slot_lo + batch);
  const int item = rem / gb, g0 = rem - item * gb;
  const StripDev* desc = plan.panel_desc + item;
  const int4* dp = reinterpret_cast<const int4*>(desc);
  const int4 d2 = __ldg(dp + 2);
  if (d2.w != PROG_RC && d2.w != PROG_CR && !(FOLD && (d2.w == PROG_MIXED || d2.w == PROG_GENERAL))) {
    for (int slot = slot_lo + g0; slot < slot_hi; slot += gb) fill_strip<false>(net, b, g, plan, desc, slot, q0, out);
    return;
  }
  if (FOLD && (d2.w == PROG_MIXED || d2.w == PROG_GENERAL) && g0 != 0) return;
  const int4 d0 = __ldg(dp), d1 = __ldg(dp + 1), d3 = __ldg(dp + 3);
  TileDev t;
  t.mat = 0;
  t.row0 = d1.y, t.nrows = d1.z, t.col0 = d1.w, t.ncols = d2.x, t.grow0 = d2.y, t.gcol0 = d2.z, t.prog = d2.w;
  t.rblk = d3.x, t.cblk = d3.y, t.flags = (uint32_t)d3.z;
  MatDev mat;
  mat.out_off = ((long long)(unsigned)d0.x) | ((long long)d0.y << 32);
  mat.ld = d1.x;
  mat.n = d3.w;
  if (FOLD && t.prog != PROG_RC && t.prog != PROG_CR) {
    emit_edge_tile(net, b, g, plan, t, mat, q0, slot_lo, slot_hi - slot_lo, out, smem);
    return;
  }
  const int slot0 = slot_lo + g0 * group;
  const int nslots = min(group, slot_hi - slot0);
  if (nslots <= 0) return;
  if (t.prog == PROG_RC) {
    if (t.ncols == FAST_TC) emit_rc<BETA, true>(net, b, plan, t, mat, q0, slot0, nslots, out, smem);
    else emit_rc<BETA, false>(net, b, plan, t, mat, q0, slot0, nslots, out, smem);
  } else {
    emit_cr<BETA>(net, b, plan, t, mat, q0, slot0, nslots, out, smem, &mbar);
  }
}

}

namespace {
__device__ __forceinline__ void band_entry(const NetDev& net, const BatchDev& b, const GramDev& g, const BandDev& bd,
                                           long long per_query, int q0, int slot, int idx, double* __restrict__ out) {
  const int q = q0 + slot, K = net.K, beta = b.beta, nt = 2 * beta + 1;
  if (idx >= bd.m * nt) return;
  const int i = idx / nt, t = idx - i * nt - beta, c = i + t;
  if (bd.upper_only && t < 0) return;
  double* o = out + (long long)slot * per_query;
  if (c < 0 || c >= bd.m) {
    if (bd.band_off >= 0 && t >= 0) o[bd.band_off + t + (long long)(beta + 1) * i] = 0.0;
    return;
  }
  const int Br = bd.blk, n0 = net.n_in;
  const long long acdim = net.acdim;
  const int rl = bd.g0 - net.off[Br] + i, cl = rl + t;
  const int jr = bd.g0 + i - n0, jc = jr + t;
  const bool copy = Br <= K - 2 && b.cnt[(long long)q * K + Br] > 0;
  const bool s22 = Br == K - 1 && b.has_s22;
  double val = 0.0;
  if (copy) val += g.scratch[(long long)slot * g.per_query + g.goff[Br] + rl + (long long)cl * g.ldG[Br]];
  if (s22) val += s22_entry(net.M[K - 1], b.U + (long long)q * net.n_out * net.n[K - 1], net.n_out, rl, cl);
  val += 0.0;
  val = __dadd_rn(val, band_term(b.T0 + (long long)q * acdim, b.gbnd + q * b.s_gbnd, b.Bt + (long long)q * beta * acdim,
                                 acdim, jr, jc));
  if (bd.ld > 0 && (!bd.optional || copy || s22)) o[bd.out_off + (bd.row0 + i) + (long long)(bd.col0 + c) * bd.ld] = val;
  if (bd.band_off >= 0 && t >= 0) o[bd.band_off + t + (long long)(beta + 1) * i] = val;
}

__global__ void __launch_bounds__(ETHREADS)
emit_band_kernel(NetDev net, BatchDev b, GramDev g, const BandDev* __restrict__ bands, long long per_query, int q0,
                 int nq, int spc, double* __restrict__ out) {
  const BandDev bd = bands[blockIdx.y];
  const int idx = blockIdx.x * ETHREADS + threadIdx.x;
  for (int slot = blockIdx.z * spc; slot < min(nq, (blockIdx.z + 1) * spc); ++slot)
    band_entry(net, b, g, bd, per_query, q0, slot, idx, out);
}
}

int launch_emit_band(const NetDev& net, const BatchDev& b, const GramDev& g, const BandDev* bands, int nbands,
                     int max_m, long long per_query, int q0, int nq, double* out, cudaStream_t st) {
  if (nbands <= 0 || nq <= 0 || max_m <= 0) return 0;
  const int nx = (max_m * (2 * b.beta + 1) + ETHREADS - 1) / ETHREADS;
  static const int spc_env = [] { const char* e = getenv("NNSDP_BAND_GROUP"); return e ? atoi(e) : 0; }();
  const int spc = spc_env > 0 ? spc_env : (nq >= 16 ? 4 : 1);
  emit_band_kernel<<<dim3(nx, nbands, (nq + spc - 1) / spc), ETHREADS, 0, st>>>(net, b, g, bands, per_query, q0, nq, spc, out);
  return 1;
}

namespace {
__global__ void pack_thin_kernel(const double* __restrict__ ring, long long per_query,
                                 const long long* __restrict__ idx, long long nthin,
                                 double* __restrict__ packed, int nq) {
  const long long total = nthin * nq;
  for (long long i = blockIdx.x * (long long)blockDim.x + threadIdx.x; i < total;
       i += (long long)gridDim.x * blockDim.x) {
    const long long s = i / nthin, k = i - s * nthin;
    packed[i] = ring[s * per_query + idx[k]];
  }
}
}

int launch_pack_thin(const double* ring, long long per_query, const long long* idx, long long nthin,
                     double* packed, int nq, cudaStream_t st) {
  if (nthin <= 0 || nq <= 0) return 0;
  long long blocks = (nthin * nq + 255) / 256;
  if (blocks > 148 * 16) blocks = 148 * 16;
  pack_thin_kernel<<<(int)blocks, 256, 0, st>>>(ring, per_query, idx, nthin, packed, nq);
  return 1;
}

static int launch_bulk(const NetDev& net, const BatchDev& b, const GramDev& g, const PlanDev& plan, int q0,
                       const BulkItem* sel, int nsel, double* out, cudaStream_t st) {
  int launches = 0;
  for (int i0 = 0; i0 < nsel; i0 += BULK_PER_LAUNCH) {
    BulkSel s;
    s.n = std::min(BULK_PER_LAUNCH, nsel - i0);
    int most = 0;
    for (int i = 0; i < s.n; ++i) {
      s.item[i] = sel[i0 + i];
      most = std::max(most, s.item[i].count);
    }
    if (most == 0) continue;
    const dim3 grid((unsigned)most, (unsigned)s.n);
    if (plan.band_inline) emit_fill_kernel<true><<<grid, ETHREADS, 0, st>>>(net, b, g, plan, q0, s, out);
    else emit_fill_kernel<false><<<grid, ETHREADS, 0, st>>>(net, b, g, plan, q0, s, out);
    ++launches;
  }
  return launches;
}

int launch_emit(const NetDev& net, const BatchDev& b, const GramDev& g, const PlanDev& plan,
                int q0, int nq, double* out, cudaStream_t st, int which, const BulkItem* sel, int nsel) {
  if (nq <= 0) return 0;
  static const int wgroup = [] { const char* e = getenv("NNSDP_WINDOW_GROUP"); int v = e ? atoi(e) : 4; return v < 1 ? 1 : (v > SLOT_GROUP ? SLOT_GROUP : v); }();
  static const int egroup_env = [] { const char* e = getenv("NNSDP_EDGE_GROUP"); int v = e ? atoi(e) : 0; return v < 0 ? 0 : (v > SLOT_GROUP ? SLOT_GROUP : v); }();
  const int egroup = egroup_env > 0 ? egroup_env : (nq >= 64 ? SLOT_GROUP : (nq >= 16 ? 4 : 1));
  int launches = 0;
  if (plan.n_panel > 0 && b.beta <= MAX_WINDOW_BETA) {
    if (which < 0 || which == 0) {
      static const int pgroup = [] { const char* e = getenv("NNSDP_PANEL_GROUP"); int v = e ? atoi(e) : 2; return v < 1 ? 1 : (v > SLOT_GROUP ? SLOT_GROUP : v); }();
      static const int pbatch_env = [] { const char* e = getenv("NNSDP_PANEL_BATCH"); return e ? atoi(e) : 8; }();
      int pbatch = std::max(pgroup, (pbatch_env / pgroup) * pgroup);
      if (pbatch > 255) pbatch = (255 / pgroup) * pgroup;
      const int nbatches = (nq + pbatch - 1) / pbatch;
      const dim3 grid((unsigned)plan.n_panel * (pbatch / pgroup) * nbatches);
      const int gp = pgroup | (pbatch << 8);
#define NNSDP_PANEL_LAUNCH(B)                                                                                  \
  if (plan.fold) emit_panel_kernel<B, true><<<grid, ETHREADS, 0, st>>>(net, b, g, plan, q0, nq, gp, out);      \
  else emit_panel_kernel<B, false><<<grid, ETHREADS, 0, st>>>(net, b, g, plan, q0, nq, gp, out);
      switch (b.beta) {
        case 0: NNSDP_PANEL_LAUNCH(0) break;
        case 1: NNSDP_PANEL_LAUNCH(1) break;
        case 2: NNSDP_PANEL_LAUNCH(2) break;
        case 3: NNSDP_PANEL_LAUNCH(3) break;
        default: NNSDP_PANEL_LAUNCH(4) break;
      }
#undef NNSDP_PANEL_LAUNCH
      ++launches;
    }
  } else {
  if (plan.n_strips > 0 && (which < 0 || which == 0)) {
    if (plan.band_inline) emit_fill_kernel<true><<<dim3(plan.n_strips, nq), ETHREADS, 0, st>>>(net, b, g, plan, q0, nq, out);
    else emit_fill_kernel<false><<<dim3(plan.n_strips, nq), ETHREADS, 0, st>>>(net, b, g, plan, q0, nq, out);
    ++launches;
  }
  if (plan.n_window > 0 && (which < 0 || which == 1)) {
    const dim3 grid(plan.n_window * ((nq + wgroup - 1) / wgroup));
    const int t0 = plan.n_fill;
    static const int gm_env = [] { const char* e = getenv("NNSDP_WINDOW_GROUP_MAJOR"); return e ? atoi(e) : -1; }();
    const int gm = gm_env >= 0 ? gm_env : plan.band_inline;
    switch (b.beta) {
      case 0: emit_window_kernel<0><<<grid, ETHREADS, 0, st>>>(net, b, plan, t0, q0, nq, wgroup, gm, out); break;
      case 1: emit_window_kernel<1><<<grid, ETHREADS, 0, st>>>(net, b, plan, t0, q0, nq, wgroup, gm, out); break;
      case 2: emit_window_kernel<2><<<grid, ETHREADS, 0, st>>>(net, b, plan, t0, q0, nq, wgroup, gm, out); break;
      case 3: emit_window_kernel<3><<<grid, ETHREADS, 0, st>>>(net, b, plan, t0, q0, nq, wgroup, gm, out); break;
      case 4: emit_window_kernel<4><<<grid, ETHREADS, 0, st>>>(net, b, plan, t0, q0, nq, wgroup, gm, out); break;
      default: return -1;
    }
    ++launches;
  }
  }
  if (which < 0 || which == 0) launches += launch_bulk(net, b, g, plan, q0, sel, nsel, out, st);
  if (!plan.fold && plan.n_edge > 0 && (which < 0 || which == 2)) {
    emit_edge_kernel<<<dim3(plan.n_edge, (nq + egroup - 1) / egroup), ETHREADS, 0, st>>>(
        net, b, g, plan, plan.n_fill + plan.n_window, q0, nq, egroup, out);
    ++launches;
  }
  return launches;
}

}
```

### nn-sdp_b200/csrc/kernels_gram.cu

```cuda
#include "internal.h"
#include <stdlib.h>

namespace nnsdp {

namespace {

constexpr int GK = 16;
constexpr int GSTAGES = 3;
#ifndef NNSDP_GRAM_WARPS_N
#define NNSDP_GRAM_WARPS_N 4
#endif
#ifndef NNSDP_GRAM_LD_PAD
#define NNSDP_GRAM_LD_PAD 4
#endif
template <int GT>
struct GramCfg {
  static constexpr int WARPS_N = GT >= 128 ? NNSDP_GRAM_WARPS_N : 2;
  static constexpr int THREADS = 4 * WARPS_N * 32;
};

template <int GT>
struct GramSmem {
  static constexpr int GLD = GT + NNSDP_GRAM_LD_PAD;
  double A[GSTAGES][GK][GLD];
  double B[GSTAGES][GK][GLD];
  double d[GSTAGES][GK];
};

__device__ __forceinline__ void cp_async16(void* smem, const void* gmem, bool valid) {
  const unsigned s = (unsigned)__cvta_generic_to_shared(smem);
  const int sz = valid ? 16 : 0;
  asm volatile("cp.async.cg.shared.global [%0], [%1], 16, %2;\n" ::"r"(s), "l"(gmem), "r"(sz));
}
__device__ __forceinline__ void cp_async_commit() { asm volatile("cp.async.commit_group;\n" ::); }
template <int N>
__device__ __forceinline__ void cp_async_wait() {
  asm volatile("cp.async.wait_group %0;\n" ::"n"(N));
}

__device__ __forceinline__ void dmma_m8n8k4(double& c0, double& c1, double a, double b) {
  asm volatile("mma.sync.aligned.m8n8k4.row.col.f64.f64.f64.f64 {%0,%1}, {%2}, {%3}, {%0,%1};\n"
               : "+d"(c0), "+d"(c1)
               : "d"(a), "d"(b));
}

template <int GT>
__global__ void __launch_bounds__(GramCfg<GT>::THREADS, 1)
gram_kernel(NetDev net, BatchDev b, GramDev g, int q0, const int* __restrict__ pairs) {
  constexpr int GTHREADS = GramCfg<GT>::THREADS;
  constexpr int GLD = GramSmem<GT>::GLD, WM = GT / 4, WN = GT / GramCfg<GT>::WARPS_N, NI = WM / 8, NJ = WN / 8;
  extern __shared__ __align__(16) unsigned char smem_raw[];
  GramSmem<GT>& sm = *reinterpret_cast<GramSmem<GT>*>(smem_raw);

  const int q = pairs[2 * blockIdx.x], blk = pairs[2 * blockIdx.x + 1], slot = q - q0;
  const int cnt = b.cnt[(long long)q * net.K + blk];
  if (cnt == 0) return;
  const int nb = net.n[blk];
  const int ntile = (nb + GT - 1) / GT;
  int ti = 0, rem = blockIdx.y;
  while (ti < ntile && rem >= ntile - ti) {
    rem -= ntile - ti;
    ++ti;
  }
  if (ti >= ntile) return;
  const int tj = ti + rem;
  const bool diag = (ti == tj);
  const int m0 = ti * GT, n0 = tj * GT;

  const double* Wt = net.Wt[blk];
  const int ldT = net.ldT[blk];
  const int L0 = net.off[blk + 1] - net.n_in;
  const int* act = b.act + (long long)q * net.acdim + L0;
  const double* d11 = b.d11 + (long long)q * net.acdim + L0;

  const int tid = threadIdx.x, lane = tid & 31, warp = tid >> 5;
  const int wm = (warp & 3) * WM, wn = (warp >> 2) * WN;
  const int nsteps = (cnt + GK - 1) / GK;

  auto load_stage = [&](int stage, int step) {
    const int k0 = step * GK;
    for (int c = tid; c < GK * (GT / 2); c += GTHREADS) {
      const int kk = c / (GT / 2), ch = c % (GT / 2);
      const bool valid = (k0 + kk) < cnt;
      const int jl = valid ? act[k0 + kk] : 0;
      const double* col = Wt + (long long)jl * ldT;
      cp_async16(&sm.A[stage][kk][ch * 2], col + m0 + ch * 2, valid);
      if (!diag) cp_async16(&sm.B[stage][kk][ch * 2], col + n0 + ch * 2, valid);
    }
    if (tid < GK) sm.d[stage][tid] = (k0 + tid < cnt) ? d11[act[k0 + tid]] : 0.0;
  };

  double acc[NI][NJ][2];
#pragma unroll
  for (int i = 0; i < NI; ++i)
#pragma unroll
    for (int j = 0; j < NJ; ++j) acc[i][j][0] = acc[i][j][1] = 0.0;

  for (int s = 0; s < GSTAGES - 1; ++s) {
    if (s < nsteps) load_stage(s, s);
    cp_async_commit();
  }
  for (int step = 0; step < nsteps; ++step) {
    cp_async_wait<GSTAGES - 2>();
    __syncthreads();
    {
      const int nxt = step + GSTAGES - 1;
      if (nxt < nsteps) load_stage(nxt % GSTAGES, nxt);
      cp_async_commit();
    }
    const int st = step % GSTAGES;
    const double(*As)[GLD] = sm.A[st];
    const double(*Bs)[GLD] = diag ? sm.A[st] : sm.B[st];
#pragma unroll
    for (int k4 = 0; k4 < GK; k4 += 4) {
      const int k = k4 + (lane & 3);
      const double dk = sm.d[st][k];
      double af[NI], bf[NJ];
#pragma unroll
      for (int i = 0; i < NI; ++i) af[i] = As[k][wm + i * 8 + (lane >> 2)] * dk;
#pragma unroll
      for (int j = 0; j < NJ; ++j) bf[j] = Bs[k][wn + j * 8 + (lane >> 2)];
#pragma unroll
      for (int i = 0; i < NI; ++i)
#pragma unroll
        for (int j = 0; j < NJ; ++j) dmma_m8n8k4(acc[i][j][0], acc[i][j][1], af[i], bf[j]);
    }
  }
  cp_async_wait<0>();

  double* G = g.scratch + (long long)slot * g.per_query + g.goff[blk];
  const int ldG = g.ldG[blk];
#pragma unroll
  for (int i = 0; i < NI; ++i) {
    const int r = m0 + wm + i * 8 + (lane >> 2);
#pragma unroll
    for (int j = 0; j < NJ; ++j) {
      const int c = n0 + wn + j * 8 + (lane & 3) * 2;
#pragma unroll
      for (int e = 0; e < 2; ++e) {
        const int cc = c + e;
        if (r < nb && cc < nb && (!diag || r <= cc)) {
          const double v = acc[i][j][e];
          G[r + (long long)cc * ldG] = v;
          if (r != cc && g.mirror) G[cc + (long long)r * ldG] = v;
        }
      }
    }
  }
}

}

template <int GT>
static void launch_gram_t(const NetDev& net, const BatchDev& b, const GramDev& g, int max_n, int q0, const int* pairs,
                          int npairs, cudaStream_t st) {
  cudaFuncSetAttribute(gram_kernel<GT>, cudaFuncAttributeMaxDynamicSharedMemorySize, (int)sizeof(GramSmem<GT>));
  const int ntile = (max_n + GT - 1) / GT;
  dim3 grid(npairs, ntile * (ntile + 1) / 2);
  gram_kernel<GT><<<grid, GramCfg<GT>::THREADS, sizeof(GramSmem<GT>), st>>>(net, b, g, q0, pairs);
}

int launch_gram(const NetDev& net, const BatchDev& b, const GramDev& g, int max_n, int q0, const int* pairs,
                int npairs, cudaStream_t st) {
  if (net.K < 2 || npairs <= 0) return 0;
  {
    const long long nt = (max_n + 127) / 128;
    if (nt * (nt + 1) / 2 > 65535) return -1;
  }
  static const int force = [] { const char* e = getenv("NNSDP_GRAM_TILE"); return e ? atoi(e) : 0; }();
  const int nt128 = (max_n + 127) / 128;
  const long long items128 = (long long)nt128 * (nt128 + 1) / 2 * npairs;
  const int nt64 = (max_n + 63) / 64;
  const long long pad128 = (long long)nt128 * (nt128 + 1) / 2 * 4, pad64 = (long long)nt64 * (nt64 + 1) / 2;
  const bool small = force ? force == 64 : (items128 < 148 || pad64 * 100 <= pad128 * 85);
  if (small) launch_gram_t<64>(net, b, g, max_n, q0, pairs, npairs, st);
  else launch_gram_t<128>(net, b, g, max_n, q0, pairs, npairs, st);
  return 1;
}

}
```

### nn-sdp_b200/csrc/plan.cpp

```cpp
#include <stdint.h>
#include <stdlib.h>

#include <algorithm>

#include "internal.h"
#include <atomic>
#include <cstring>
#include <thread>

namespace nnsdp {

int64_t lambda_dim(int64_t acdim, int64_t beta) {
  int64_t s = 0;
  for (int64_t t = acdim - beta; t <= acdim; ++t) s += t;
  return s;
}

long long gram_layout(const Shape& sh, std::vector<long long>* goff, std::vector<int>* ldG) {
  goff->assign(sh.K, 0);
  ldG->assign(sh.K, 0);
  long long go = 0;
  for (int blk = 0; blk <= sh.K - 2; ++blk) {
    (*ldG)[blk] = (int)(((sh.n[blk] + 15) / 16) * 16);
    (*goff)[blk] = go;
    go += (long long)(*ldG)[blk] * sh.n[blk];
  }
  return go;
}

static int64_t Sfun(const Shape& sh, int64_t k) {
  int64_t s = 0;
  for (int64_t i = 0; i < k; ++i) s += sh.n[i];
  return s;
}

int32_t make_cliques_host(const Shape& sh, int64_t beta, CliqueInfoHost* out) {
  const int K = sh.K;
  out->ck.clear();
  out->d1.clear();
  out->d2.clear();
  int64_t p = 1;
  for (int64_t i = 1; i <= K; ++i) {
    if (Sfun(sh, i + 1) + beta >= Sfun(sh, K - 1)) {
      p = i;
      break;
    }
  }
  for (int64_t k = 1; k <= p - 1; ++k) {
    CliqueRanges c;
    c.nseg = 2;
    c.lo[0] = Sfun(sh, k - 1);
    c.hi[0] = Sfun(sh, k + 1) + beta - 1;
    c.lo[1] = Sfun(sh, K - 1);
    c.hi[1] = Sfun(sh, K);
    NN_CHECK(c.hi[0] <= c.lo[1], NNSDP_ERR_ASSERT,
             "makeCliques: Ck1[end] <= Ck2[1] violated (chordal_cliques.jl:35)");
    NN_CHECK(c.hi[0] < c.lo[1], NNSDP_ERR_ASSERT, "makeCliques: Ck1 and Ck2 overlap");
    const int64_t ckdim = c.size();
    std::vector<int64_t> d1, d2;
    if (k == 1) {
      for (int64_t i = 1; i <= ckdim; ++i) d1.push_back(i);
    } else {
      const int64_t nk = sh.n[k - 1], nk1 = sh.n[k];
      for (int64_t i = 1; i <= nk + nk1 + beta; ++i) d1.push_back(i);
      d1.push_back(ckdim);
      for (int64_t i = nk + nk1 + 1; i <= ckdim; ++i) d2.push_back(i);
    }
    out->ck.push_back(c);
    out->d1.push_back(d1);
    out->d2.push_back(d2);
  }
  CliqueRanges c;
  c.nseg = 1;
  c.lo[0] = Sfun(sh, p - 1);
  c.hi[0] = Sfun(sh, K);
  std::vector<int64_t> d1;
  for (int64_t i = 1; i <= c.size(); ++i) d1.push_back(i);
  out->ck.push_back(c);
  out->d1.push_back(d1);
  out->d2.push_back({});
  return NNSDP_OK;
}

int32_t fill_sizes(const Shape& sh, int64_t beta, nnsdp_sizes* s) {
  NN_CHECK(beta >= 0, NNSDP_ERR_ASSERT, "QcActivSector: 0 <= beta violated (activ_sector.jl:12)");
  NN_CHECK(beta <= sh.acdim, NNSDP_ERR_ASSERT,
           "QcActivSector: acxdim + length(ijs) == _lambda_dim needs beta <= acxdim "
           "(activ_sector.jl:18,32)");
  CliqueInfoHost ci;
  NN_TRY(make_cliques_host(sh, beta, &ci));
  s->K = sh.K;
  s->Zdim = sh.Zdim;
  s->acdim = sh.acdim;
  s->xtot = sh.xtot;
  s->lamdim = lambda_dim(sh.acdim, beta);
  s->secdim = s->lamdim + 2 * sh.acdim;
  s->n_in = sh.n_in();
  s->n_out = sh.n_out();
  s->sdim = sh.n_in() + sh.n_out() + 1;
  s->ncliques = (int64_t)ci.ck.size();
  s->sum_ck = s->sum_ck_sq = s->sum_dk = s->max_ck = 0;
  for (size_t k = 0; k < ci.ck.size(); ++k) {
    const int64_t n = ci.ck[k].size();
    s->sum_ck += n;
    s->sum_ck_sq += n * n;
    s->sum_dk += (int64_t)(ci.d1[k].size() + ci.d2[k].size());
    s->max_ck = std::max(s->max_ck, n);
  }
  return NNSDP_OK;
}

int32_t build_chol_plan(const Shape& sh, const std::vector<CliqueRanges>& mats, std::vector<CholFront>* fronts) {
  const int p = (int)mats.size();
  NN_CHECK(p >= 1, NNSDP_ERR_ASSERT, "certify plan: no clique");
  std::vector<std::vector<int64_t>> idx(p);
  std::vector<int> owner(sh.Zdim, -1);
  for (int k = 0; k < p; ++k) {
    for (int s = 0; s < mats[k].nseg; ++s)
      for (int64_t g = mats[k].lo[s]; g <= mats[k].hi[s]; ++g) idx[k].push_back(g);
    for (int64_t g : idx[k]) {
      NN_CHECK(g >= 0 && g < sh.Zdim, NNSDP_ERR_ASSERT, "certify plan: index %lld outside Z", (long long)g);
      owner[g] = k;
    }
  }
  for (int64_t g = 0; g < sh.Zdim; ++g)
    NN_CHECK(owner[g] >= 0, NNSDP_ERR_ASSERT, "certify plan: index %lld lies in no clique", (long long)g);
  fronts->assign(p, CholFront{});
  std::vector<uint8_t> shifted(sh.Zdim, 0);
  long long off = 0;
  for (int k = 0; k < p; ++k) {
    CholFront& f = (*fronts)[k];
    const std::vector<int64_t>& c = idx[k];
    f.out_off = off;
    f.n = (int)c.size();
    off += (long long)f.n * f.n;
    int np = 0;
    while (np < f.n && owner[c[np]] == k) ++np;
    f.npriv = np;
    f.g0 = c[0];
    for (int i = 0; i < f.n; ++i) {
      NN_CHECK((owner[c[i]] == k) == (i < np), NNSDP_ERR_ASSERT,
               "certify plan: the private indices of clique %d are not a leading range", k + 1);
      if (i < np)
        NN_CHECK(c[i] == f.g0 + i, NNSDP_ERR_ASSERT, "certify plan: private indices of clique %d not contiguous", k + 1);
    }
    NN_CHECK(np >= 1, NNSDP_ERR_ASSERT, "certify plan: clique %d has no private index", k + 1);
    NN_CHECK(k + 1 < p || np == f.n, NNSDP_ERR_ASSERT, "certify plan: the last clique is not all private");
    if (k > 0) {
      const CholFront& pf = (*fronts)[k - 1];
      const std::vector<int64_t>& pc = idx[k - 1];
      const int ns = pf.n - pf.npriv;
      const int seg1 = (int)(mats[k - 1].hi[0] - mats[k - 1].lo[0] + 1);
      f.lead = seg1 - pf.npriv;
      f.tail = ns - f.lead;
      NN_CHECK(f.lead >= 0 && f.tail >= 0 && f.lead + f.tail <= f.n, NNSDP_ERR_ASSERT,
               "certify plan: separator of cliques %d, %d does not fit", k, k + 1);
      for (int s = 0; s < ns; ++s) {
        const int li = s < f.lead ? s : f.n - (ns - s);
        NN_CHECK(c[li] == pc[pf.npriv + s], NNSDP_ERR_ASSERT,
                 "certify plan: index %lld of clique %d is not at its place in clique %d", (long long)pc[pf.npriv + s], k,
                 k + 1);
      }
    }
    for (int i = f.lead; i < f.n - f.tail; ++i) {
      NN_CHECK(!shifted[c[i]], NNSDP_ERR_ASSERT, "certify plan: diagonal entry %lld shifted twice", (long long)c[i]);
      shifted[c[i]] = 1;
    }
  }
  for (int64_t g = 0; g < sh.Zdim; ++g)
    NN_CHECK(shifted[g], NNSDP_ERR_ASSERT, "certify plan: diagonal entry %lld never shifted", (long long)g);
  return NNSDP_OK;
}

namespace {

struct Piece {
  int64_t g0, g1;
  int64_t l0;
};

// ... 255 lines not shown
    }
    std::stable_sort(strips.begin(), strips.end(), [](const TileDev& x, const TileDev& y) {
      if (x.mat != y.mat) return x.mat < y.mat;
      if (x.col0 != y.col0) return x.col0 < y.col0;
      return x.row0 < y.row0;
    });
    std::stable_sort(rowjobs.begin(), rowjobs.end(), [](const TileDev& x, const TileDev& y) {
      if (x.mat != y.mat) return x.mat < y.mat;
      return x.col0 < y.col0;
    });
    for (size_t i = 0; i < rowjobs.size();) {
      TileDev m = rowjobs[i];
      size_t j = i + 1;
      for (; j < rowjobs.size(); ++j) {
        const TileDev& n = rowjobs[j];
        if (n.mat != m.mat || n.row0 != m.row0 || n.col0 != m.col0 + m.ncols || n.gcol0 != m.gcol0 + m.ncols ||
            m.ncols + n.ncols > AFFROW_COLS)
          break;
        m.ncols += n.ncols;
      }
      strips.push_back(m);
      i = j;
    }
    plan->tiles = strips;
    plan->tiles.insert(plan->tiles.end(), rest.begin(), rest.end());
  }
  if (packed) {
    std::vector<TileDev> keep;
    for (const TileDev& t : plan->tiles)
      if (!strictly_lower(t)) keep.push_back(t);
    plan->tiles.swap(keep);
    PackedLayout& L = *packed;
    L = PackedLayout();
    L.diag_cell.assign(K, -1);
    L.diag_entries.assign(K, 0);
    std::vector<PackedCell> rect, band, window, diag;
    auto is_diag_strip = [&](const TileDev& t) {
      return (t.prog == PROG_SAME || t.prog == PROG_DIAG) && cls(t) == 0 && t.rblk >= 1 && t.rblk == t.cblk;
    };
    auto inside = [](const TileDev& t, const PackedCell& c) {
      return t.grow0 >= c.grow0 && t.grow0 + t.nrows <= c.grow0 + c.nrows && t.gcol0 >= c.gcol0 &&
             t.gcol0 + t.ncols <= c.gcol0 + c.ncols;
    };
    if (split_blocks) {
      for (int b = 0; b <= K - 2; ++b)
        window.push_back({PK_WINDOW, b, sh.off[b], sh.off[b + 1], sh.n[b], sh.n[b + 1], 0, 1});
      std::vector<int64_t> lo(K, sh.Zdim), hi(K, -1);
      for (const TileDev& t : plan->tiles)
        if (is_diag_strip(t)) {
          lo[t.rblk] = std::min<int64_t>(lo[t.rblk], std::min(t.grow0, t.gcol0));
          hi[t.rblk] = std::max<int64_t>(hi[t.rblk], std::max(t.grow0 + t.nrows, t.gcol0 + t.ncols) - 1);
        }
      for (int b = 1; b <= K - 1; ++b)
        if (hi[b] >= lo[b]) {
          const int64_t m = hi[b] - lo[b] + 1;
          diag.push_back({PK_DIAG, b, lo[b], lo[b], m, m, 0, 0});
          band.push_back({PK_BAND, b, lo[b], lo[b], beta + 1, m, 0, 1});
        }
    }
    auto find_cell = [&](const TileDev& t, int* which) -> int {
      if (is_diag_strip(t)) {
        for (size_t i = 0; i < diag.size(); ++i)
          if (diag[i].blk == t.rblk && inside(t, diag[i])) { *which = PK_DIAG; return (int)i; }
      } else {
        for (size_t i = 0; i < window.size(); ++i)
          if (inside(t, window[i])) { *which = PK_WINDOW; return (int)i; }
      }
      return -1;
    };
    std::vector<int> left;
    for (size_t i = 0; i < plan->tiles.size(); ++i) {
      int which = 0;
      if (find_cell(plan->tiles[i], &which) < 0) left.push_back((int)i);
    }
    if (!split_blocks) {
      rect.push_back({PK_RECT, -1, 0, 0, sh.Zdim, sh.Zdim, 0, 1});
    } else {
      std::sort(left.begin(), left.end(), [&](int x, int y) {
        const TileDev &a = plan->tiles[x], &b2 = plan->tiles[y];
        if (a.gcol0 != b2.gcol0) return a.gcol0 < b2.gcol0;
        if (a.ncols != b2.ncols) return a.ncols < b2.ncols;
        return a.grow0 < b2.grow0;
      });
      for (int i : left) {
        const TileDev& t = plan->tiles[i];
        if (!rect.empty()) {
          PackedCell& c = rect.back();
          if (c.gcol0 == t.gcol0 && c.ncols == t.ncols && c.grow0 + c.nrows == t.grow0) {
            c.nrows += t.nrows;
            continue;
          }
        }
        rect.push_back({PK_RECT, -1, t.grow0, t.gcol0, t.nrows, t.ncols, 0, 1});
      }
      std::sort(rect.begin(), rect.end(), [](const PackedCell& a, const PackedCell& b2) {
        if (a.grow0 != b2.grow0) return a.grow0 < b2.grow0;
        if (a.nrows != b2.nrows) return a.nrows < b2.nrows;
        return a.gcol0 < b2.gcol0;
      });
      std::vector<PackedCell> merged;
      for (const PackedCell& c : rect) {
        if (!merged.empty()) {
          PackedCell& m = merged.back();
          if (m.grow0 == c.grow0 && m.nrows == c.nrows && m.gcol0 + m.ncols == c.gcol0) {
            m.ncols += c.ncols;
            continue;
          }
        }
        merged.push_back(c);
      }
      rect.swap(merged);
    }
    int64_t off = 0;
    auto place = [&](std::vector<PackedCell>& v) {
      for (PackedCell& c : v) {
        c.offset = off;
        off += ((c.nrows * c.ncols + 15) / 16) * 16;
        L.cells.push_back(c);
      }
    };
    place(rect);
    place(band);
    place(window);
    L.always_doubles = off;
    const size_t first_diag = L.cells.size();
    place(diag);
    L.record_doubles = off;
    for (size_t i = first_diag; i < L.cells.size(); ++i) L.diag_cell[L.cells[i].blk] = (int32_t)i;
    const size_t first_window = rect.size() + band.size();
    plan->mats.clear();
    for (const PackedCell& c : L.cells) plan->mats.push_back({c.offset, (int32_t)c.nrows, (int32_t)c.nrows});
    for (TileDev& t : plan->tiles) {
      int which = 0, ci = find_cell(t, &which), cell = -1;
      if (ci >= 0) {
        cell = (int)((which == PK_DIAG ? first_diag : first_window) + ci);
      } else {
        for (size_t i = 0; i < rect.size() && cell < 0; ++i)
          if (inside(t, L.cells[i])) cell = (int)i;
      }
      NN_CHECK(cell >= 0, NNSDP_ERR_STATE, "packed plan: a tile lies in no cell");
      const PackedCell& c = L.cells[cell];
      t.mat = cell;
      t.row0 = (int32_t)(t.grow0 - c.grow0);
      t.col0 = (int32_t)(t.gcol0 - c.gcol0);
      if (c.kind == PK_DIAG) L.diag_entries[c.blk] += (int64_t)t.nrows * t.ncols;
      else L.always_entries += (int64_t)t.nrows * t.ncols;
    }
    for (const PackedCell& c : band) L.always_entries += c.nrows * c.ncols;
    plan->per_query_doubles = L.record_doubles;
  }
  std::stable_sort(plan->tiles.begin(), plan->tiles.end(),
                   [&](const TileDev& x, const TileDev& y) { return cls(x) < cls(y); });
  {
    std::vector<long long> goff;
    std::vector<int> ldG;
    gram_layout(sh, &goff, &ldG);
    plan->strips.clear();
    for (const TileDev& t : plan->tiles) {
      if (cls(t) != 0) break;
      StripDev d{};
      d.out_off = plan->mats[t.mat].out_off;
      d.ld = plan->mats[t.mat].ld;
      d.row0 = t.row0; d.nrows = t.nrows; d.col0 = t.col0; d.ncols = t.ncols;
      d.grow0 = t.grow0; d.gcol0 = t.gcol0; d.prog = t.prog; d.rblk = t.rblk;
      if ((t.prog == PROG_SAME || t.prog == PROG_DIAG) && t.rblk >= 0) {
        d.rl0 = (int32_t)(t.grow0 - sh.off[t.rblk] - t.row0);
        d.cl0 = (int32_t)(t.gcol0 - sh.off[t.rblk]);
        if (t.rblk <= K - 2) {
          d.goff = goff[t.rblk];
          d.ldG = ldG[t.rblk];
        }
      }
      plan->strips.push_back(d);
    }
  }
  {
    plan->bands.clear();
    struct Box { int64_t lo = INT64_MAX, hi = -1, l0 = 0; bool band = false; };
    std::vector<std::vector<Box>> box(plan->mats.size(), std::vector<Box>(K));
    int64_t widest = 0;
    for (const TileDev& t : plan->tiles) {
      if (cls(t) != 0 || !(t.prog == PROG_SAME || t.prog == PROG_DIAG) || t.rblk < 1 || t.rblk != t.cblk) continue;
      Box& bx = box[t.mat][t.rblk];
      const int64_t lo = std::min<int64_t>(t.grow0, t.gcol0);
      if (lo < bx.lo) {
        bx.lo = lo;
        bx.l0 = (t.grow0 <= t.gcol0) ? t.row0 : t.col0;
      }
      bx.hi = std::max<int64_t>(bx.hi, std::max<int64_t>(t.grow0 + t.nrows, t.gcol0 + t.ncols) - 1);
      bx.band |= (t.prog == PROG_DIAG);
      widest = std::max<int64_t>(widest, bx.hi - bx.lo + 1);
    }
    plan->band_inline = widest < 256;
    for (size_t m = 0; m < plan->mats.size(); ++m)
      for (int blk = 1; blk < K; ++blk) {
        const Box& bx = box[m][blk];
        if (bx.hi < bx.lo || !bx.band) continue;
        BandDev j{};
        j.out_off = plan->mats[m].out_off;
        j.band_off = -1;
        j.ld = plan->band_inline ? 0 : plan->mats[m].ld;
        j.row0 = j.col0 = (int)bx.l0;
        j.g0 = (int)bx.lo;
        j.m = (int)(bx.hi - bx.lo + 1);
        j.blk = blk;
        if (packed) {
          const PackedCell& c = packed->cells[m];
          j.optional = (c.kind == PK_DIAG);
          j.upper_only = 1;
          for (const PackedCell& bc : packed->cells)
            if (bc.kind == PK_BAND && bc.blk == blk) j.band_off = bc.offset;
        }
        if (j.ld > 0 || j.band_off >= 0) plan->bands.push_back(j);
      }
  }
  plan->n_fill = plan->n_window = plan->n_edge = 0;
  for (const TileDev& t : plan->tiles) {
    const int c = cls(t);
    (c == 0 ? plan->n_fill : c == 1 ? plan->n_window : plan->n_edge)++;
  }
  plan->panel.clear();
  plan->panel_fold.clear();
  if (!packed && !plan->band_inline && plan->n_window > 0 && beta <= MAX_WINDOW_BETA) {
    struct Key { long long off; int panel, row0, col0; StripDev d; };
    std::vector<Key> keys;
    auto sorted = [](std::vector<Key> k) {
      std::stable_sort(k.begin(), k.end(), [](const Key& x, const Key& y) {
        if (x.off != y.off) return x.off < y.off;
        if (x.panel != y.panel) return x.panel < y.panel;
        if (x.col0 != y.col0) return x.col0 < y.col0;
        return x.row0 < y.row0;
      });
      std::vector<StripDev> v(k.size());
      for (size_t i = 0; i < k.size(); ++i) v[i] = k[i].d;
      return v;
    };
    auto add_tile = [&](const TileDev& t) {
      const MatDev& m = plan->mats[t.mat];
      StripDev d{};
      d.out_off = m.out_off;
      d.ld = m.ld;
      d.row0 = t.row0; d.nrows = t.nrows; d.col0 = t.col0; d.ncols = t.ncols;
      d.grow0 = t.grow0; d.gcol0 = t.gcol0; d.prog = t.prog;
      d.rblk = t.rblk; d.rl0 = t.cblk; d.cl0 = (int32_t)t.flags; d.ldG = m.n;
      keys.push_back({d.out_off, d.col0 / 32, d.row0, d.col0, d});
    };
    for (int i = 0; i < plan->n_fill; ++i) {
      const StripDev& d = plan->strips[i];
      keys.push_back({d.out_off, d.col0 / 32, d.row0, d.col0, d});
    }
    for (int i = 0; i < plan->n_window; ++i) add_tile(plan->tiles[plan->n_fill + i]);
    plan->panel = sorted(keys);
    for (int i = 0; i < plan->n_edge; ++i) add_tile(plan->tiles[plan->n_fill + plan->n_window + i]);
    plan->panel_fold = sorted(keys);
  }
  return NNSDP_OK;
}


static void unpack_one(int64_t beta, const PackedLayout& lay, const CliqueRanges& ck, const double* record,
                       const uint8_t* present, double* o) {
  const int64_t n = ck.size();
  std::memset(o, 0, (size_t)n * n * sizeof(double));
  constexpr int64_t TB = 64;
  auto copy_rect = [&](const PackedCell& c) {
    const double* src = record + c.offset;
    int64_t rbase = 0;
    for (int sr = 0; sr < ck.nseg; rbase += ck.hi[sr] - ck.lo[sr] + 1, ++sr) {
      const int64_t r0 = std::max(c.grow0, ck.lo[sr]), r1 = std::min(c.grow0 + c.nrows - 1, ck.hi[sr]);
      if (r0 > r1) continue;
      int64_t cbase = 0;
      for (int sc = 0; sc < ck.nseg; cbase += ck.hi[sc] - ck.lo[sc] + 1, ++sc) {
        const int64_t c0 = std::max(c.gcol0, ck.lo[sc]), c1 = std::min(c.gcol0 + c.ncols - 1, ck.hi[sc]);
        if (c0 > c1 || r0 > c1) continue;
        const int64_t lr_of = rbase - ck.lo[sr], lc_of = cbase - ck.lo[sc];
        for (int64_t gcb = std::max(c0, r0); gcb <= c1; gcb += TB) {
          const int64_t gce = std::min(gcb + TB - 1, c1);
          for (int64_t grb = r0; grb <= std::min(r1, gce); grb += TB) {
            const int64_t gre = std::min(grb + TB - 1, r1);
            for (int64_t gc = gcb; gc <= gce; ++gc) {
              const int64_t rhi = std::min(gre, gc);
              if (grb > rhi) continue;
              const double* col = src + (gc - c.gcol0) * c.nrows - c.grow0;
              std::memcpy(o + (lr_of + grb) + (lc_of + gc) * n, col + grb, (size_t)(rhi - grb + 1) * sizeof(double));
            }
            for (int64_t gr = grb; gr <= gre; ++gr) {
              const int64_t glo = std::max(gcb, gr);
              if (glo > gce) continue;
              double* dst = o + (lr_of + gr) * n + lc_of;
              const double* s0 = src - c.grow0 + gr - c.gcol0 * c.nrows;
              for (int64_t gc = glo; gc <= gce; ++gc) dst[gc] = s0[gc * c.nrows];
            }
          }
        }
      }
    }
  };
  auto local = [&](int64_t g) -> int64_t {
    int64_t base = 0;
    for (int s = 0; s < ck.nseg; base += ck.hi[s] - ck.lo[s] + 1, ++s)
      if (g >= ck.lo[s] && g <= ck.hi[s]) return base + g - ck.lo[s];
    return -1;
  };
  for (int pass : {PK_DIAG, PK_WINDOW, PK_BAND, PK_RECT})
    for (size_t i = 0; i < lay.cells.size(); ++i) {
      const PackedCell& c = lay.cells[i];
      if (c.kind != pass || !present[i]) continue;
      if (c.kind != PK_BAND) {
        copy_rect(c);
        continue;
      }
      const double* src = record + c.offset;
      for (int64_t j = 0; j < c.ncols; ++j) {
        const int64_t lr = local(c.grow0 + j);
        if (lr < 0) continue;
        for (int64_t t = 0; t <= beta && j + t < c.ncols; ++t) {
          const int64_t lc = local(c.grow0 + j + t);
          if (lc < 0) continue;
          const double v = src[t + (beta + 1) * j];
          o[lr + lc * n] = v;
          o[lc + lr * n] = v;
        }
      }
    }
// ... 119 lines not shown
```

Before: 9463.

## Compact Gram scratch per active pair and batch Gram launches across chunks

Gram scratch is now laid out compactly: each (query, block) pair with nonzero active count gets its own offset in a per-query offset table, replacing the fixed per-query stride. One Gram launch can cover as many queries as fit in a configurable memory budget and is reused by later emit chunks, so fewer Gram launches are issued. Small hidden blocks (n ≤ 8) are computed by a per-warp DMMA path inside the same kernel instead of occupying full tiles. The changes add host-side table construction and a scratch buffer whose size depends on the budget, and they change the addressing in every emit kernel.

```diff
diff --git a/nn-sdp_b200/csrc/api.cu b/nn-sdp_b200/csrc/api.cu
--- a/nn-sdp_b200/csrc/api.cu
+++ b/nn-sdp_b200/csrc/api.cu
@@ -198,9 +198,11 @@
   cudaEvent_t ev_packed[GATHER_STAGES] = {nullptr, nullptr, nullptr, nullptr};
   std::unique_ptr<WorkerPool> pool;
   std::vector<int> h_cnt;
-  std::vector<int> h_pairs;
-  std::vector<int64_t> pair_begin;
-  DevBuf d_pairs;
+  std::vector<int64_t> wide_begin, small_begin, gram_pre;
+  DevBuf d_gram_list;
+  const int* d_pairs = nullptr;
+  int64_t gram_q0 = 0, gram_q1 = 0;
+  int64_t gram_budget = 0;
   int64_t gather_bytes_dma = 0, gather_bytes_zeroed = 0, gather_bytes_thin = 0;
   nnsdp_ctx* ctx = nullptr;
   int dev_index = 0, dev = 0;
@@ -225,10 +227,8 @@
   DevBuf ze_netv, ze_g, ze_rows, ze_part, ze_io, ze_err;
   nnsdp_sizes sz{};
   PlanHost plan;
-  DevBuf d_tiles, d_strips, d_bulk, d_mats, d_panel, d_goff, d_ldG;
-  std::vector<long long> goff;
+  DevBuf d_tiles, d_strips, d_bulk, d_mats, d_panel, d_ldG;
   std::vector<int> ldG;
-  long long gram_per_query = 0;
   DevBuf x1min, x1max, ymin, ymax, smin, smax, gin, gbnd, gsec, outS, outvec, outinvP, gout;
   DevBuf xmin, xmax, acxmin, acxmax, smin_c, smax_c;
   DevBuf d11, Md, T0, Bt, u, aff, part, act, cnt, Z11, Z1K, U;
@@ -287,7 +287,7 @@
     spans.clear();
   }
   std::vector<DevBuf*> all_bufs() {
-    return {&d_bands, &d_tmaps, &d_tmap_ok, &d_tiles, &d_strips, &d_bulk, &d_mats, &d_panel, &d_goff, &d_ldG, &d_chol, &ze_netv, &ze_g, &ze_rows, &ze_part, &ze_io, &ze_err, &x1min, &x1max, &ymin, &ymax, &smin, &smax,
+    return {&d_bands, &d_tmaps, &d_tmap_ok, &d_tiles, &d_strips, &d_bulk, &d_mats, &d_panel, &d_ldG, &d_chol, &ze_netv, &ze_g, &ze_rows, &ze_part, &ze_io, &ze_err, &x1min, &x1max, &ymin, &ymax, &smin, &smax,
             &gin, &gbnd, &gsec, &outS, &outvec, &outinvP, &gout, &xmin, &xmax, &acxmin, &acxmax,
             &smin_c, &smax_c, &d11, &Md, &T0, &Bt, &u, &aff, &part, &act, &cnt, &Z11, &Z1K, &U,
             &gram, &ringbuf, &flags, &cr_rowsA, &cr_rowsB, &cr_bias, &cr_prel, &cr_preu, &cr_du, &cr_bu, &cr_dl,
@@ -721,7 +721,7 @@
   for (DevBuf* x : b->all_bufs()) x->release();
   b->d_thin_idx.release();
   b->d_packed.release();
-  b->d_pairs.release();
+  b->d_gram_list.release();
   if (b->h_packed) cudaFreeHost(b->h_packed);
   for (cudaEvent_t e : b->ev_packed)
     if (e) cudaEventDestroy(e);
@@ -798,11 +798,12 @@
     NN_TRY(b->Z1K.ensure((size_t)sh.n_in() * sh.n[sh.K - 1] * Q * 8));
     NN_TRY(b->U.ensure((size_t)sh.n_out() * sh.n[sh.K - 1] * Q * 8));
     b->bd.npart = npart;
-    const long long go = gram_layout(sh, &b->goff, &b->ldG);
-    b->gram_per_query = go;
-    NN_TRY(upload(b->d_goff, b->goff.data(), b->goff.size() * 8, b->st));
+    {
+      const char* e = getenv("NNSDP_GRAM_BUDGET_MB");
+      b->gram_budget = (int64_t)std::max(0LL, e ? atoll(e) : 8192LL) << 17;
+    }
+    b->ldG = gram_ld(sh);
     NN_TRY(upload(b->d_ldG, b->ldG.data(), b->ldG.size() * 4, b->st));
-    NN_TRY(b->gram.ensure((size_t)go * b->ring * 8));
     std::vector<CliqueRanges> mats;
     NN_TRY(format_mats(sh, beta, dense_Z, &mats));
     const char* noclass = getenv("NNSDP_NO_TILE_CLASSES");
@@ -922,9 +923,6 @@
     }
     b->pd.packed = b->plan.skip_absent ? 1 : 0;
     b->pd.band_inline = b->plan.band_inline ? 1 : 0;
-    b->gd.scratch = b->gram.as<double>();
-    b->gd.per_query = go;
-    b->gd.goff = b->d_goff.as<long long>();
     b->gd.ldG = b->d_ldG.as<int>();
     b->gd.mirror = b->packed && b->plan.skip_absent ? 0 : 1;
   }
@@ -1125,20 +1123,42 @@
   b->h_cnt.resize((size_t)sh.K * b->Q);
   NN_CUDA(cudaMemcpyAsync(b->h_cnt.data(), b->cnt.p, b->h_cnt.size() * 4, cudaMemcpyDeviceToHost, b->st));
   NN_TRY(check_flags(b, "nnsdp_batch_prepare"));
-  b->h_pairs.clear();
-  b->pair_begin.assign((size_t)b->Q + 1, 0);
-  for (int64_t q = 0; q < b->Q; ++q) {
-    for (int blk = 0; blk <= sh.K - 2; ++blk)
-      if (b->h_cnt[(size_t)q * sh.K + blk] > 0) {
-        b->h_pairs.push_back((int)q);
-        b->h_pairs.push_back(blk);
-      }
-    b->pair_begin[q + 1] = (int64_t)b->h_pairs.size() / 2;
-  }
-  NN_TRY(upload(b->d_pairs, b->h_pairs.data(), b->h_pairs.size() * 4, b->st));
   const BatchDev& bd = b->bd;
   b->shared_gram = b->Q > 1 && bd.s_gsec == 0 &&
                    (b->bounds_supplied ? (bd.s_smin == 0 && bd.s_smax == 0) : (bd.s_x1min == 0 && bd.s_x1max == 0));
+  {
+    const int64_t nq = b->shared_gram ? 1 : b->Q;
+    const bool tiles_only = gram_force_tiles();
+    std::vector<int> wide, small;
+    std::vector<long long> qoff((size_t)sh.K * b->Q, -1);
+    b->wide_begin.assign((size_t)nq + 1, 0);
+    b->small_begin.assign((size_t)nq + 1, 0);
+    b->gram_pre.assign((size_t)nq + 1, 0);
+    int64_t off = 0;
+    for (int64_t q = 0; q < nq; ++q) {
+      for (int blk = 0; blk <= sh.K - 2; ++blk)
+        if (b->h_cnt[(size_t)q * sh.K + blk] > 0) {
+          std::vector<int>& v = (sh.n[blk] <= GRAM_SMALL_N && !tiles_only) ? small : wide;
+          v.push_back((int)q);
+          v.push_back(blk);
+          qoff[(size_t)q * sh.K + blk] = off;
+          off += (int64_t)b->ldG[blk] * sh.n[blk];
+        }
+      b->wide_begin[q + 1] = (int64_t)wide.size() / 2;
+      b->small_begin[q + 1] = (int64_t)small.size() / 2;
+      b->gram_pre[q + 1] = off;
+    }
+    for (int64_t q = nq; q < b->Q; ++q)
+      std::copy(qoff.begin(), qoff.begin() + sh.K, qoff.begin() + q * sh.K);
+    const size_t ntab = qoff.size();
+    wide.insert(wide.end(), small.begin(), small.end());
+    qoff.resize(ntab + (wide.size() + 1) / 2);
+    memcpy(qoff.data() + ntab, wide.data(), wide.size() * 4);
+    NN_TRY(upload(b->d_gram_list, qoff.data(), qoff.size() * 8, b->st));
+    b->gd.qoff = b->d_gram_list.as<long long>();
+    b->d_pairs = reinterpret_cast<const int*>(b->gd.qoff + ntab);
+    b->gram_q0 = b->gram_q1 = 0;
+  }
   b->prepared = true;
   return NNSDP_OK;
 }
@@ -1198,6 +1218,33 @@
   return NNSDP_OK;
 }
 
+static int32_t gram_for(nnsdp_batch* b, int64_t q0, int64_t nq, GramDev* gd) {
+  const int64_t budget = b->gram_budget;
+  if (b->shared_gram) q0 = 0, nq = 1;
+  const int64_t nown = (int64_t)b->gram_pre.size() - 1;
+  if (q0 < b->gram_q0 || q0 + nq > b->gram_q1) {
+    int64_t q1 = q0 + nq;
+    while (q1 < nown && b->gram_pre[q1 + 1] - b->gram_pre[q0] <= budget) ++q1;
+    b->gram_q0 = b->gram_q1 = 0;
+    NN_TRY(b->gram.ensure((size_t)(b->gram_pre[q1] - b->gram_pre[q0]) * 8));
+    GramDev g = b->gd;
+    g.scratch = b->gram.as<double>() - b->gram_pre[q0];
+    const int64_t w0 = b->wide_begin[q0], w1 = b->wide_begin[q1], s0 = b->small_begin[q0], s1 = b->small_begin[q1];
+    const int* pairs = b->d_pairs;
+    b->span_begin(ST_GRAM, b->st);
+    const int l = launch_gram(b->nd->nd, b->bd, g, (int)b->net->max_block, pairs + 2 * w0, (int)(w1 - w0),
+                              pairs + 2 * (b->wide_begin[nown] + s0), (int)(s1 - s0), b->st);
+    b->span_end(b->st, std::max(l, 0));
+    NN_CHECK(l >= 0, NNSDP_ERR_ARG, "a hidden layer of %lld neurons is too wide for the Gram kernel's grid",
+             (long long)b->net->max_block);
+    NN_CUDA(cudaGetLastError());
+    b->gram_q0 = q0, b->gram_q1 = q1;
+  }
+  *gd = b->gd;
+  gd->scratch = b->gram.as<double>() - b->gram_pre[b->gram_q0];
+  return NNSDP_OK;
+}
+
 int32_t nnsdp_batch_emit(nnsdp_batch* b, int64_t q0, int64_t nq) {
   NN_CHECK(b != nullptr, NNSDP_ERR_ARG, "batch is NULL");
   NN_CHECK(b->prepared, NNSDP_ERR_STATE, "nnsdp_batch_emit before nnsdp_batch_prepare");
@@ -1205,20 +1252,8 @@
            "bad query range [%lld, %lld) for Q = %lld, ring = %lld", (long long)q0,
            (long long)(q0 + nq), (long long)b->Q, (long long)b->ring);
   NN_CUDA(cudaSetDevice(b->dev));
-  const NetPerDev& nd = *b->nd;
-  GramDev gd = b->gd;
-  b->span_begin(ST_GRAM, b->st);
-  int l;
-  if (b->shared_gram) {
-    l = launch_gram(nd.nd, b->bd, gd, (int)b->net->max_block, 0, b->d_pairs.as<int>(), (int)b->pair_begin[1], b->st);
-    gd.per_query = 0;
-  } else {
-    l = launch_gram(nd.nd, b->bd, gd, (int)b->net->max_block, (int)q0, b->d_pairs.as<int>() + 2 * b->pair_begin[q0],
-                    (int)(b->pair_begin[q0 + nq] - b->pair_begin[q0]), b->st);
-  }
-  b->span_end(b->st, l > 0 ? l : 0);
-  NN_CHECK(l >= 0, NNSDP_ERR_ARG, "a hidden layer of %lld neurons is too wide for the Gram kernel's grid", (long long)b->net->max_block);
-  NN_CUDA(cudaGetLastError());
+  GramDev gd;
+  NN_TRY(gram_for(b, q0, nq, &gd));
   NN_TRY(emit_pass(b, gd, (int)q0, (int)nq, b->ringbuf.as<double>()));
   return NNSDP_OK;
 }
@@ -1394,22 +1429,11 @@
   for (int64_t q0 = 0; q0 < b->Q && status == NNSDP_OK; q0 += chunk, h = (h + 1) % nhalf, ++ci) {
     const int64_t nq = std::min(chunk, b->Q - q0);
     double* dst = b->ringbuf.as<double>() + (int64_t)h * chunk * per;
-    GramDev gd = b->gd;
-    if (b->shared_gram) gd.per_query = 0;
-    else gd.scratch += (int64_t)h * chunk * gd.per_query;
     if (sparse && ci >= GATHER_STAGES) b->pool->wait_group(ci - GATHER_STAGES);
     if (host_out && used[h]) NN_CUDA(cudaStreamWaitEvent(b->st, b->ev_free[h], 0));
-    if (!b->shared_gram || ci == 0) {
-      b->span_begin(ST_GRAM, b->st);
-      int l = b->shared_gram
-                  ? launch_gram(nd.nd, b->bd, b->gd, (int)b->net->max_block, 0, b->d_pairs.as<int>(), (int)b->pair_begin[1], b->st)
-                  : launch_gram(nd.nd, b->bd, gd, (int)b->net->max_block, (int)q0, b->d_pairs.as<int>() + 2 * b->pair_begin[q0],
-                                (int)(b->pair_begin[q0 + nq] - b->pair_begin[q0]), b->st);
-      b->span_end(b->st, l > 0 ? l : 0);
-      NN_CHECK(l >= 0, NNSDP_ERR_ARG, "a hidden layer of %lld neurons is too wide for the Gram kernel's grid",
-               (long long)b->net->max_block);
-      NN_CUDA(cudaGetLastError());
-    }
+    GramDev gd;
+    status = gram_for(b, q0, nq, &gd);
+    if (status != NNSDP_OK) break;
     status = emit_pass(b, gd, (int)q0, (int)nq, dst);
     if (status != NNSDP_OK) break;
     if (sparse) {
diff --git a/nn-sdp_b200/csrc/internal.h b/nn-sdp_b200/csrc/internal.h
--- a/nn-sdp_b200/csrc/internal.h
+++ b/nn-sdp_b200/csrc/internal.h
@@ -66,7 +66,7 @@
 
 int32_t make_cliques_host(const Shape& sh, int64_t beta, CliqueInfoHost* out);
 int64_t lambda_dim(int64_t acdim, int64_t beta);
-long long gram_layout(const Shape& sh, std::vector<long long>* goff, std::vector<int>* ldG);
+std::vector<int> gram_ld(const Shape& sh);
 int32_t fill_sizes(const Shape& sh, int64_t beta, nnsdp_sizes* out);
 
 enum TileFlags : uint32_t {
@@ -98,7 +98,7 @@
 
 struct alignas(16) StripDev {
   long long out_off;
-  long long goff;
+  long long reserved;
   int32_t ld, row0, nrows, col0;
   int32_t ncols, grow0, gcol0, prog;
   int32_t rblk, rl0, cl0, ldG;
@@ -234,8 +234,7 @@
 
 struct GramDev {
   double* scratch;
-  long long per_query;
-  const long long* goff;
+  const long long* qoff;
   const int* ldG;
   int mirror;
 };
@@ -288,8 +287,10 @@
 int launch_transpose_w(const double* Mk, int n_out_k, int n_in_k, double* Wt, int ldT,
                        cudaStream_t st);
 int launch_prep(const NetDev& net, const BatchDev& b, int* err_flag, cudaStream_t st);
-int launch_gram(const NetDev& net, const BatchDev& b, const GramDev& g, int max_n, int q0, const int* pairs,
-                int npairs, cudaStream_t st);
+constexpr int GRAM_SMALL_N = 8;
+bool gram_force_tiles();
+int launch_gram(const NetDev& net, const BatchDev& b, const GramDev& g, int max_n, const int* pairs, int nwide,
+                const int* small, int nsmall, cudaStream_t st);
 struct BulkItem {
   int32_t slot, first, count;
 };
diff --git a/nn-sdp_b200/csrc/kernels_emit.cu b/nn-sdp_b200/csrc/kernels_emit.cu
--- a/nn-sdp_b200/csrc/kernels_emit.cu
+++ b/nn-sdp_b200/csrc/kernels_emit.cu
@@ -24,11 +24,10 @@
   const double* Z1K;
   const double* U;
   const int* cnt;
-  const double* G;
+  const long long* goff;
 };
 
-__device__ __forceinline__ QView make_view(const NetDev& net, const BatchDev& b, const GramDev& g,
-                                           int q, int slot) {
+__device__ __forceinline__ QView make_view(const NetDev& net, const BatchDev& b, const GramDev& g, int q) {
   const long long acdim = net.acdim;
   const int K = net.K, n0 = net.n_in;
   QView v;
@@ -41,7 +40,7 @@
   v.Z1K = b.Z1K + (long long)q * n0 * net.n[K - 1];
   v.U = b.U + (long long)q * net.n_out * net.n[K - 1];
   v.cnt = b.cnt + (long long)q * K;
-  v.G = g.scratch + (long long)slot * g.per_query;
+  v.goff = g.qoff + (long long)q * K;
   return v;
 }
 
@@ -98,7 +97,7 @@
   if (tr >= t.nrows) return;
 
   const int rl = rl0 + tr, jr = jr0 + tr;
-  const double* Gp = gram ? v.G + g.goff[Br] + rl : nullptr;
+  const double* Gp = gram ? g.scratch + v.goff[Br] + rl : nullptr;
   const int ldG = gram ? g.ldG[Br] : 0;
   const double* WtR = rc ? net.Wt[Br] + rl : nullptr;
   const int ldTR = rc ? net.ldT[Br] : 0;
@@ -173,7 +172,7 @@
       const int cl = gc - net.off[Bc];
       const int jc = gc >= n0 ? gc - n0 : -1;
       if ((flags & TF_SAME) && Br == Bc) {
-        if (Br <= K - 2 && v.cnt[Br] > 0) val += v.G[g.goff[Br] + rl + (long long)cl * g.ldG[Br]];
+        if (Br <= K - 2 && v.cnt[Br] > 0) val += g.scratch[v.goff[Br] + rl + (long long)cl * g.ldG[Br]];
         if (Br == 0) val += v.Z11[rl + cl * n0];
         if (Br == K - 1 && b.has_s22) {
           const int lo = rl < cl ? rl : cl, hi = rl < cl ? cl : rl;
@@ -449,13 +448,12 @@
   }
   const int4 d3 = __ldg(dp + 3);
   const int Br = d3.x, rl0 = d3.y, cl0 = d3.z, ldG = d3.w;
-  const long long goff = ((long long)(unsigned)d0.z) | ((long long)d0.w << 32);
   const bool copy = Br <= K - 2 && b.cnt[(long long)q * K + Br] > 0;
   const bool s22 = Br == K - 1 && b.has_s22;
   if (plan.packed && !copy && !s22) return;
   const double* WK = net.M[K - 1];
   const double* U = b.U + (long long)q * net.n_out * net.n[K - 1];
-  const double* G = g.scratch + (long long)slot * g.per_query + goff + rl0;
+  const double* G = g.scratch + (copy ? g.qoff[(long long)q * K + Br] : 0) + rl0;
   if (BAND_INLINE && prog == PROG_DIAG) {
     const int beta = b.beta;
     const long long acdim = net.acdim;
@@ -546,7 +544,7 @@
   const bool uniform = (t.flags & TF_UNIFORM) != 0 && t.nrows * t.ncols > 512;
   if (uniform) {
     for (int s = 0; s < nslots; ++s) {
-      const QView v = make_view(net, b, g, q0 + slot0 + s, slot0 + s);
+      const QView v = make_view(net, b, g, q0 + slot0 + s);
       double* o = out + (long long)(slot0 + s) * plan.per_query + tile_off;
       emit_mixed(net, b, g, t, mat, v, o, tr, cg, ncg, smem);
     }
@@ -558,7 +556,7 @@
   const int spar = ETHREADS / per;
   const int sub = threadIdx.x / per, cg2 = (threadIdx.x % per) / TR;
   for (int s = sub; s < nslots; s += spar) {
-    const QView v = make_view(net, b, g, q0 + slot0 + s, slot0 + s);
+    const QView v = make_view(net, b, g, q0 + slot0 + s);
     double* o = out + (long long)(slot0 + s) * plan.per_query + tile_off;
     emit_general(net, b, g, t, mat, v, o, tr, cg2, TC);
   }
@@ -642,7 +640,7 @@
   const bool copy = Br <= K - 2 && b.cnt[(long long)q * K + Br] > 0;
   const bool s22 = Br == K - 1 && b.has_s22;
   double val = 0.0;
-  if (copy) val += g.scratch[(long long)slot * g.per_query + g.goff[Br] + rl + (long long)cl * g.ldG[Br]];
+  if (copy) val += g.scratch[g.qoff[(long long)q * K + Br] + rl + (long long)cl * g.ldG[Br]];
   if (s22) val += s22_entry(net.M[K - 1], b.U + (long long)q * net.n_out * net.n[K - 1], net.n_out, rl, cl);
   val += 0.0;
   val = __dadd_rn(val, band_term(b.T0 + (long long)q * acdim, b.gbnd + q * b.s_gbnd, b.Bt + (long long)q * beta * acdim,
diff --git a/nn-sdp_b200/csrc/kernels_gram.cu b/nn-sdp_b200/csrc/kernels_gram.cu
--- a/nn-sdp_b200/csrc/kernels_gram.cu
+++ b/nn-sdp_b200/csrc/kernels_gram.cu
@@ -44,15 +44,62 @@
                : "d"(a), "d"(b));
 }
 
+__device__ __forceinline__ void gram_small_pair(const NetDev& net, const BatchDev& b, const GramDev& g, const int* pairs,
+                                                int p) {
+  const int lane = threadIdx.x & 31;
+  const int q = pairs[2 * p], blk = pairs[2 * p + 1];
+  const int cnt = b.cnt[(long long)q * net.K + blk];
+  if (cnt == 0) return;
+  const int nb = net.n[blk];
+  const double* Wt = net.Wt[blk];
+  const int ldT = net.ldT[blk];
+  const int L0 = net.off[blk + 1] - net.n_in;
+  const int* act = b.act + (long long)q * net.acdim + L0;
+  const double* d11 = b.d11 + (long long)q * net.acdim + L0;
+  const int r = lane >> 2, kl = lane & 3;
+  double c0 = 0.0, c1 = 0.0;
+  const int kend = (cnt + GK - 1) / GK * GK;
+  for (int k0 = 0; k0 < kend; k0 += GK) {
+    double a[GK / 4], w[GK / 4];
+#pragma unroll
+    for (int i = 0; i < GK / 4; ++i) {
+      const int k = k0 + 4 * i + kl;
+      const bool valid = k < cnt;
+      const int j = valid ? act[k] : 0;
+      w[i] = (valid && r < nb) ? Wt[(long long)j * ldT + r] : 0.0;
+      a[i] = valid ? d11[j] : 0.0;
+    }
+#pragma unroll
+    for (int i = 0; i < GK / 4; ++i) dmma_m8n8k4(c0, c1, w[i] * a[i], w[i]);
+  }
+  double* G = g.scratch + g.qoff[(long long)q * net.K + blk];
+  const int ldG = g.ldG[blk];
+#pragma unroll
+  for (int e = 0; e < 2; ++e) {
+    const int cc = kl * 2 + e;
+    if (r < nb && cc < nb && r <= cc) {
+      const double v = e ? c1 : c0;
+      G[r + (long long)cc * ldG] = v;
+      if (r != cc && g.mirror) G[cc + (long long)r * ldG] = v;
+    }
+  }
+}
+
 template <int GT>
 __global__ void __launch_bounds__(GramCfg<GT>::THREADS, 1)
-gram_kernel(NetDev net, BatchDev b, GramDev g, int q0, const int* __restrict__ pairs) {
+gram_kernel(NetDev net, BatchDev b, GramDev g, const int* __restrict__ pairs, int nwide, const int* __restrict__ small,
+            int nsmall) {
   constexpr int GTHREADS = GramCfg<GT>::THREADS;
   constexpr int GLD = GramSmem<GT>::GLD, WM = GT / 4, WN = GT / GramCfg<GT>::WARPS_N, NI = WM / 8, NJ = WN / 8;
   extern __shared__ __align__(16) unsigned char smem_raw[];
   GramSmem<GT>& sm = *reinterpret_cast<GramSmem<GT>*>(smem_raw);
-
-  const int q = pairs[2 * blockIdx.x], blk = pairs[2 * blockIdx.x + 1], slot = q - q0;
+  if ((int)blockIdx.x >= nwide) {
+    const int p = ((int)blockIdx.x - nwide) * (GTHREADS / 32) + (int)(threadIdx.x >> 5);
+    if (blockIdx.y == 0 && p < nsmall) gram_small_pair(net, b, g, small, p);
+    return;
+  }
+
+  const int q = pairs[2 * blockIdx.x], blk = pairs[2 * blockIdx.x + 1];
   const int cnt = b.cnt[(long long)q * net.K + blk];
   if (cnt == 0) return;
   const int nb = net.n[blk];
@@ -128,7 +175,7 @@
   }
   cp_async_wait<0>();
 
-  double* G = g.scratch + (long long)slot * g.per_query + g.goff[blk];
+  double* G = g.scratch + g.qoff[(long long)q * net.K + blk];
   const int ldG = g.ldG[blk];
 #pragma unroll
   for (int i = 0; i < NI; ++i) {
@@ -152,29 +199,36 @@
 }
 
 template <int GT>
-static void launch_gram_t(const NetDev& net, const BatchDev& b, const GramDev& g, int max_n, int q0, const int* pairs,
-                          int npairs, cudaStream_t st) {
+static void launch_gram_t(const NetDev& net, const BatchDev& b, const GramDev& g, int max_n, const int* pairs, int nwide,
+                          const int* small, int nsmall, cudaStream_t st) {
   cudaFuncSetAttribute(gram_kernel<GT>, cudaFuncAttributeMaxDynamicSharedMemorySize, (int)sizeof(GramSmem<GT>));
-  const int ntile = (max_n + GT - 1) / GT;
-  dim3 grid(npairs, ntile * (ntile + 1) / 2);
-  gram_kernel<GT><<<grid, GramCfg<GT>::THREADS, sizeof(GramSmem<GT>), st>>>(net, b, g, q0, pairs);
-}
-
-int launch_gram(const NetDev& net, const BatchDev& b, const GramDev& g, int max_n, int q0, const int* pairs,
-                int npairs, cudaStream_t st) {
-  if (net.K < 2 || npairs <= 0) return 0;
+  const int ntile = (max_n + GT - 1) / GT, per = GramCfg<GT>::THREADS / 32;
+  dim3 grid(nwide + (nsmall + per - 1) / per, nwide > 0 ? ntile * (ntile + 1) / 2 : 1);
+  gram_kernel<GT><<<grid, GramCfg<GT>::THREADS, sizeof(GramSmem<GT>), st>>>(net, b, g, pairs, nwide, small, nsmall);
+}
+
+static int gram_force() {
+  static const int force = [] { const char* e = getenv("NNSDP_GRAM_TILE"); return e ? atoi(e) : 0; }();
+  return force;
+}
+
+bool gram_force_tiles() { return gram_force() != 0; }
+
+int launch_gram(const NetDev& net, const BatchDev& b, const GramDev& g, int max_n, const int* pairs, int nwide,
+                const int* small, int nsmall, cudaStream_t st) {
+  if (net.K < 2 || nwide + nsmall <= 0) return 0;
   {
     const long long nt = (max_n + 127) / 128;
     if (nt * (nt + 1) / 2 > 65535) return -1;
   }
-  static const int force = [] { const char* e = getenv("NNSDP_GRAM_TILE"); return e ? atoi(e) : 0; }();
+  const int force = gram_force();
   const int nt128 = (max_n + 127) / 128;
-  const long long items128 = (long long)nt128 * (nt128 + 1) / 2 * npairs;
+  const long long items128 = (long long)nt128 * (nt128 + 1) / 2 * nwide;
   const int nt64 = (max_n + 63) / 64;
   const long long pad128 = (long long)nt128 * (nt128 + 1) / 2 * 4, pad64 = (long long)nt64 * (nt64 + 1) / 2;
-  const bool small = force ? force == 64 : (items128 < 148 || pad64 * 100 <= pad128 * 85);
-  if (small) launch_gram_t<64>(net, b, g, max_n, q0, pairs, npairs, st);
-  else launch_gram_t<128>(net, b, g, max_n, q0, pairs, npairs, st);
+  const bool small64 = force ? force == 64 : (items128 < 148 || pad64 * 100 <= pad128 * 85);
+  if (small64) launch_gram_t<64>(net, b, g, max_n, pairs, nwide, small, nsmall, st);
+  else launch_gram_t<128>(net, b, g, max_n, pairs, nwide, small, nsmall, st);
   return 1;
 }
 
diff --git a/nn-sdp_b200/csrc/plan.cpp b/nn-sdp_b200/csrc/plan.cpp
--- a/nn-sdp_b200/csrc/plan.cpp
+++ b/nn-sdp_b200/csrc/plan.cpp
@@ -16,16 +16,10 @@
   return s;
 }
 
-long long gram_layout(const Shape& sh, std::vector<long long>* goff, std::vector<int>* ldG) {
-  goff->assign(sh.K, 0);
-  ldG->assign(sh.K, 0);
-  long long go = 0;
-  for (int blk = 0; blk <= sh.K - 2; ++blk) {
-    (*ldG)[blk] = (int)(((sh.n[blk] + 15) / 16) * 16);
-    (*goff)[blk] = go;
-    go += (long long)(*ldG)[blk] * sh.n[blk];
-  }
-  return go;
+std::vector<int> gram_ld(const Shape& sh) {
+  std::vector<int> ldG(sh.K, 0);
+  for (int blk = 0; blk <= sh.K - 2; ++blk) ldG[blk] = (int)(((sh.n[blk] + 15) / 16) * 16);
+  return ldG;
 }
 
 static int64_t Sfun(const Shape& sh, int64_t k) {
@@ -587,9 +581,7 @@
   std::stable_sort(plan->tiles.begin(), plan->tiles.end(),
                    [&](const TileDev& x, const TileDev& y) { return cls(x) < cls(y); });
   {
-    std::vector<long long> goff;
-    std::vector<int> ldG;
-    gram_layout(sh, &goff, &ldG);
+    const std::vector<int> ldG = gram_ld(sh);
     plan->strips.clear();
     for (const TileDev& t : plan->tiles) {
       if (cls(t) != 0) break;
@@ -601,10 +593,7 @@
       if ((t.prog == PROG_SAME || t.prog == PROG_DIAG) && t.rblk >= 0) {
         d.rl0 = (int32_t)(t.grow0 - sh.off[t.rblk] - t.row0);
         d.cl0 = (int32_t)(t.gcol0 - sh.off[t.rblk]);
-        if (t.rblk <= K - 2) {
-          d.goff = goff[t.rblk];
-          d.ldG = ldG[t.rblk];
-        }
+        if (t.rblk <= K - 2) d.ldG = ldG[t.rblk];
       }
       plan->strips.push_back(d);
     }
```

Result: faster. 9616 (median of 6 runs) (+1.6%).
